# abeytheo/gan-inpainting

Measured on AMD Instinct MI355X. Metric: training images/sec at 256x256 bs=32/GPU, higher is better.
Workload: dtype f16; 1 GPU; wgan_rmse 256x256 bs=32/GPU (BASELINE.json configs[3]): U-Net G (41.8M) + PatchGAN critic, RMSprop 5e-5, clip 0.01, RMSE recon, G update every 5th batch, random-init weights; global_batch=32, parallelism=dp1, compute=fp16 MFMA, fp32 accumulate, fp32 master weights

## Files before the change

### gan-inpainting_amd/backend.py

```python
import ctypes as C
import os
import threading

import torch

_HERE = os.path.dirname(os.path.abspath(__file__))
LIB_PATH = os.environ.get("GI_LIB_PATH") or os.path.join(_HERE, "libganinpaint.so")

GI_F32, GI_F16 = 0, 1
ACT_NONE, ACT_RELU, ACT_LRELU = 0, 1, 2

_vp, _i, _i64, _f, _u64 = C.c_void_p, C.c_int, C.c_int64, C.c_float, C.c_uint64

PROTOTYPES = {
    "gi_last_error": (C.c_char_p, []),
    "gi_version": (_i, []),
    "gi_set_option": (_i, [C.c_char_p, _i]),
    "gi_get_option": (_i, [C.c_char_p, C.POINTER(_i)]),
    "gi_debug_last_kernel": (C.c_char_p, []),
    "gi_debug_fold_count": (_i, []),
    "gi_ctx_create": (_i, [_i, _vp, C.POINTER(_vp)]),
    "gi_ctx_destroy": (_i, [_vp]),
    "gi_ctx_sync": (_i, [_vp]),
    "gi_unet_create": (_i, [_vp, _i, _i, _f, _i, _i, _i, _i, _i, C.POINTER(_vp)]),
    "gi_unet_create_ex": (_i, [_vp, _i, _i, _i, _f, _i, _i, _i, _i, _i, C.POINTER(_vp)]),
    "gi_unet_create_norm": (_i, [_vp, _i, _i, _i, _i, _f, _i, _i, _i, _i, _i, C.POINTER(_vp)]),
    "gi_unet_create_padded": (_i, [_vp, _i, _i, _i, _i, _i, _f, _i, _i, _i, _i, _i, C.POINTER(_vp)]),
    "gi_patchgan_create": (_i, [_vp, _i, _i, _i, _i, _i, _i, C.POINTER(_vp)]),
    "gi_patchgan_create_sn": (_i, [_vp, _i, _i, _i, _i, _i, _i, _i, _i, C.POINTER(_vp)]),
    "gi_net_sn_read": (_i, [_vp, _i, _vp, _vp, _i64]),
    "gi_dcgan_create": (_i, [_vp, _i, _i, _i, _i, _i, C.POINTER(_vp)]),
    "gi_dcgan_debug_forward_convs": (_i, [_vp, _i, _vp, _i]),
    "gi_net_destroy": (_i, [_vp]),
    "gi_net_tensor_count": (_i, [_vp]),
    "gi_net_tensor_desc": (_i, [_vp, _i, C.c_char_p, _i, C.POINTER(_i), C.POINTER(_i64), C.POINTER(_i),
                                C.POINTER(_i64), C.POINTER(_i64)]),
    "gi_net_param_floats": (_i64, [_vp]),
    "gi_net_buffer_floats": (_i64, [_vp]),
    "gi_net_workspace_bytes": (_i64, [_vp]),
    "gi_net_bind": (_i, [_vp, _vp, _vp, _vp, _vp, _i64]),
    "gi_net_sync_weights": (_i, [_vp]),
    "gi_net_set_train": (_i, [_vp, _i]),
    "gi_net_set_inference": (_i, [_vp, _i]),
    "gi_net_set_loss_scale": (_i, [_vp, _f]),
    "gi_net_set_bn_groups": (_i, [_vp, _i]),
    "gi_net_set_dropout_seed": (_i, [_vp, _u64]),
    "gi_net_get_dropout_state": (_i, [_vp, C.POINTER(_u64), C.POINTER(_u64)]),
    "gi_net_set_dropout_state": (_i, [_vp, _u64, _u64]),
    "gi_net_dropout_mask": (_i, [_vp, _i, _i, _vp, _i64]),
    "gi_net_saved_activation": (_i, [_vp, _i, _i, _i, _vp, _i64]),
    "gi_net_debug_nonzero_tickets": (_i, [_vp, _vp]),
    "gi_net_set_dropout_mask": (_i, [_vp, _i, _i, _vp]),
    "gi_net_forward": (_i, [_vp, _i, _vp, _vp, _i]),
    "gi_net_backward": (_i, [_vp, _i, _vp, _vp, _i]),
    "gi_net_backward_phase": (_i, [_vp, _i, _vp, _vp, _i, _i]),
    "gi_net_phase_split": (_i64, [_vp]),
    "gi_net_phase_split2": (_i64, [_vp]),
    "gi_comm_unique_id": (_i, [C.c_char_p]),
    "gi_comm_create": (_i, [C.c_char_p, _i, _i, _i, C.POINTER(_vp)]),
    "gi_comm_destroy": (_i, [_vp]),
    "gi_allreduce_sum_f32": (_i, [_vp, _vp, _i64, _vp]),
    "gi_net_allreduce_grads_async": (_i, [_vp, _vp, _i64, _i64, _vp]),
    "gi_allreduce_wait": (_i, [_vp, _vp, _vp]),
    "gi_patchgan_gradient_penalty": (_i, [_vp, _vp, _i, _f, _vp]),
    "gi_patchgan_gp_saved_activation": (_i, [_vp, _i, _vp, _i64]),
    "gi_interpolate": (_i, [_vp, _vp, _vp, _vp, _i, _i64, _vp]),
    "gi_mask_apply": (_i, [_vp, _vp, _vp, _vp, _vp, _i64, _i]),
    "gi_mask_composite": (_i, [_vp, _vp, _vp, _vp, _vp, _i64]),
    "gi_mul": (_i, [_vp, _vp, _vp, _vp, _i64]),
    "gi_add": (_i, [_vp, _vp, _vp, _vp, _i64, _f]),
    "gi_loss_l1": (_i, [_vp, _vp, _vp, _i64, _vp, _vp, _f, _vp]),
    "gi_loss_rmse": (_i, [_vp, _vp, _vp, _i64, _f, _vp, _vp, _f, _vp]),
    "gi_loss_mse": (_i, [_vp, _vp, _vp, _i64, _vp, _vp, _f, _vp]),
    "gi_loss_local": (_i, [_vp, _vp, _vp, _vp, _i64, _i, _vp, _vp, _f, _vp]),
    "gi_loss_adv": (_i, [_vp, _vp, _i, _i, _f, _vp, _vp, _f]),
    "gi_loss_adv_pair": (_i, [_vp, _vp, _i, _i, _f, _f, _vp, _vp, _vp, _f, _f]),
    "gi_adam_step": (_i, [_vp, _vp, _vp, _vp, _vp, _i64, _f, _f, _f, _f, _i, _f]),
    "gi_rmsprop_step": (_i, [_vp, _vp, _vp, _vp, _i64, _f, _f, _f, _f, _f]),
    "gi_clamp": (_i, [_vp, _vp, _i64, _f, _f]),
    "gi_grad_absmean": (_i, [_vp, _vp, _vp, _vp, _i, _vp]),
    "gi_ssim_scratch_floats": (_i64, [_i, _i, _i, _i, _i]),
    "gi_ssim": (_i, [_vp, _vp, _vp, _i, _i, _i, _i, _i, _vp, _vp, _vp, _vp]),
    "gi_eval_recon_scratch_floats": (_i64, [_i64]),
    "gi_eval_recon": (_i, [_vp, _vp, _vp, _vp, _i64, _f, _vp, _vp, _vp, _vp]),
    "gi_seg_metrics": (_i, [_vp, _vp, _vp, _i, _i, _i64, _vp, _i, _vp, _vp, _vp]),
    "gi_loss_tv": (_i, [_vp, _vp, _i, _i, _i, _f, _vp, _vp, _f, _vp]),
    "gi_loss_cross_entropy": (_i, [_vp, _vp, _vp, _i, _i, _i64, _vp, _i, _vp, _vp, _f, _vp]),
    "gi_vgg19_create": (_i, [_vp, _i, _i, _i, _vp]),
    "gi_vgg19_destroy": (None, [_vp]),
    "gi_vgg19_param_floats": (_i64, [_vp]),
    "gi_vgg19_workspace_bytes": (_i64, [_vp]),
    "gi_vgg19_num_tensors": (_i, [_vp]),
    "gi_vgg19_tensor_desc": (_i, [_vp, _i, _vp, _i, _vp, _vp]),
    "gi_vgg19_bind": (_i, [_vp, _vp, _vp, _i64]),
    "gi_vgg19_sync_weights": (_i, [_vp]),
    "gi_vgg19_perceptual_style": (_i, [_vp, _vp, _vp, _i, _f, _f, _vp, _vp]),
    "gi_vgg19_features": (_i, [_vp, _vp, _i, _i, _vp]),
    "gi_vgg19_grad_workspace_bytes": (_i64, [_vp]),
    "gi_vgg19_bind_grad": (_i, [_vp, _vp, _i64]),
    "gi_vgg19_perceptual_style_grad": (_i, [_vp, _vp, _vp, _i, _f, _f, _vp, _vp, _vp, _f]),
    "gi_vgg19_grad_layer": (_i, [_vp, _i, _vp]),
    "gi_inception_create": (_i, [_vp, _i, _i, _vp]),
    "gi_inception_destroy": (None, [_vp]),
# ... 206 lines not shown
```

### gan-inpainting_amd/csrc/api.hip

```cpp
#include <string.h>

#include <stdlib.h>

#include "common.h"
#include "stat_acc.h"
#include "igemm_plan.h"

static thread_local char g_err[1024] = "";

void gi_set_error(const char* fmt, ...) {
  va_list ap;
  va_start(ap, fmt);
  vsnprintf(g_err, sizeof(g_err), fmt, ap);
  va_end(ap);
}

namespace {
struct OptDesc { const char* name; int dflt; int value; int state; };
inline int opt_load(const int& v) { return __atomic_load_n(&v, __ATOMIC_RELAXED); }
inline void opt_store(int& v, int x) { __atomic_store_n(&v, x, __ATOMIC_RELAXED); }
OptDesc g_opts[GI_OPT_COUNT] = {
  {"GI_IGEMM5", 7, 0, 0}, {"GI_IGEMM6", 1, 0, 0}, {"GI_IGEMM7", 1, 0, 0}, {"GI_IGEMM_FIXUP", 1, 0, 0}, {"GI_IGEMM_VARIANT", 3, 0, 0},
  {"GI_BN_ACC", 1, 0, 0}, {"GI_FUSE_HEAD", 1, 0, 0}, {"GI_HEAD_FAST", 1, 0, 0}, {"GI_BN_BWD_FUSE", 1, 0, 0}, {"GI_BN_BWD_SMALL", 512, 0, 0},
  {"GI_WGRAD2", 1, 0, 0}, {"GI_WGRAD3", 1, 0, 0}, {"GI_IGEMM8", 1, 0, 0}, {"GI_BN_FOLD", 0, 0, 0}, {"GI_C1_FUSED", 1, 0, 0},
  {"GI_WGRAD_STREAM", 1, 0, 0}, {"GI_MASK_BITS", 1, 0, 0}, {"GI_C1W_FUSE", 1, 0, 0}, {"GI_IGEMM7_WAVES", 8, 0, 0},
};
thread_local const char* g_last_kernel = "";
int g_fold_count = 0;
}
void gi_note_fold() { __atomic_fetch_add(&g_fold_count, 1, __ATOMIC_RELAXED); }

int gi_opt(int id) {
  OptDesc& o = g_opts[id];
  if (opt_load(o.state) == 0) {
    const char* e = getenv(o.name);
    opt_store(o.value, e ? atoi(e) : o.dflt);
    __atomic_store_n(&o.state, 1, __ATOMIC_RELEASE);
  }
  return opt_load(o.value);
}
void gi_note_kernel(const char* name) { g_last_kernel = name; }

extern "C" {

int gi_set_option(const char* name, int value) {
  GI_REQUIRE(name, "set_option: null name");
  for (int i = 0; i < GI_OPT_COUNT; ++i)
    if (strcmp(name, g_opts[i].name) == 0) {
      if (value < 0) opt_store(g_opts[i].state, 0);
      else { opt_store(g_opts[i].value, value); __atomic_store_n(&g_opts[i].state, 2, __ATOMIC_RELEASE); }
      return GI_OK;
    }
  gi_set_error("set_option: unknown option '%s'", name);
  return GI_ERR_INVALID;
}
int gi_get_option(const char* name, int* value) {
  GI_REQUIRE(name && value, "get_option: null argument");
  for (int i = 0; i < GI_OPT_COUNT; ++i)
    if (strcmp(name, g_opts[i].name) == 0) { *value = gi_opt(i); return GI_OK; }
  gi_set_error("get_option: unknown option '%s'", name);
  return GI_ERR_INVALID;
}
const char* gi_debug_last_kernel(void) { return g_last_kernel; }
int gi_debug_fold_count(void) { return __atomic_load_n(&g_fold_count, __ATOMIC_RELAXED); }

const char* gi_last_error(void) { return g_err; }
int gi_version(void) { return 100; }

int gi_ctx_create(int device_id, void* hip_stream, gi_ctx** out) {
  GI_REQUIRE(out != nullptr, "ctx_create: out is null");
  int count = 0;
  GI_HIP(hipGetDeviceCount(&count));
  GI_REQUIRE(device_id >= 0 && device_id < count, "ctx_create: device %d not present (%d visible)", device_id, count);
  GI_HIP(hipSetDevice(device_id));
  hipDeviceProp_t prop;
  GI_HIP(hipGetDeviceProperties(&prop, device_id));
  if (strncmp(prop.gcnArchName, "gfx950", 6) != 0) {
    gi_set_error("ctx_create: device %d is %s; this library is built for gfx950 only", device_id, prop.gcnArchName);
    return GI_ERR_UNSUPPORTED;
  }
  gi_ctx* c = new gi_ctx();
  c->device = device_id;
  c->stream = (hipStream_t)hip_stream;
  *out = c;
  return GI_OK;
}
int gi_ctx_destroy(gi_ctx* ctx) {
  if (ctx && ctx->tickets) (void)hipFree(ctx->tickets);
  if (ctx && ctx->absmean_partials) (void)hipFree(ctx->absmean_partials);
  if (ctx && ctx->diffaug_partials) (void)hipFree(ctx->diffaug_partials);
  delete ctx;
  return GI_OK;
}
int gi_ctx_sync(gi_ctx* ctx) {
  GI_REQUIRE(ctx, "ctx_sync: null");
  GI_HIP(hipStreamSynchronize(ctx->stream));
  return GI_OK;
}

static unsigned* ctx_tickets(gi_ctx* ctx) {
  if (!ctx->tickets) {
    if (hipMalloc((void**)&ctx->tickets, GI_IGEMM_TICKETS * 4) != hipSuccess) { ctx->tickets = nullptr; return nullptr; }
    if (hipMemset(ctx->tickets, 0, GI_IGEMM_TICKETS * 4) != hipSuccess) { (void)hipFree(ctx->tickets); ctx->tickets = nullptr; }
  }
  return ctx->tickets;
}

int gi_conv_s2_forward(gi_ctx* ctx, int dtype, const void* in, const void* w_packed, void* out, int n, int H, int W, int cb, int ldin,
                       int ca, int ldout, int relu_in, int act_out, float* ws, int64_t ws_bytes) {
  GI_REQUIRE(ctx && in && w_packed && out, "conv_s2_forward: null pointer");
  GI_REQUIRE(H % 2 == 0 && W % 2 == 0, "conv_s2_forward: H=%d W=%d must be even", H, W);
  IgemmArgs a;
  memset(&a, 0, sizeof(a));
  a.in = in; a.w = w_packed; a.out = out; a.ws = ws; a.ws_bytes = ws_bytes;
  a.tickets = ws ? ctx_tickets(ctx) : nullptr;
  a.n = n; a.Hs = H / 2; a.Ws = W / 2;
  a.cin = cb; a.ldin = ldin; a.cout = ca; a.ldout = ldout;
  a.relu_in = relu_in; a.act_out = act_out;
  return op_igemm(ctx->stream, dtype, 0, a);
}

int gi_convT_s2_forward(gi_ctx* ctx, int dtype, const void* in, const void* w_phase, void* out, int n, int H, int W, int ca, int ldin,
                        int cb, int ldout, int relu_in, int act_out, float* ws, int64_t ws_bytes) {
  GI_REQUIRE(ctx && in && w_phase && out, "convT_s2_forward: null pointer");
  IgemmArgs a;
  memset(&a, 0, sizeof(a));
  a.in = in; a.w = w_phase; a.out = out; a.ws = ws; a.ws_bytes = ws_bytes;
  a.tickets = ws ? ctx_tickets(ctx) : nullptr;
  a.n = n; a.Hs = H; a.Ws = W;
  a.cin = ca; a.ldin = ldin; a.cout = cb; a.ldout = ldout;
  a.relu_in = relu_in; a.act_out = act_out;
  return op_igemm(ctx->stream, dtype, 1, a);
}

static int apply_ex(IgemmArgs& a, const gi_igemm_ex* ex) {
  if (!ex) return GI_OK;
  GI_REQUIRE(ex->relu_cend >= 0 && ex->relu_cend % 64 == 0 && ex->relu_cend <= a.cin, "igemm_ex: relu_cend=%d must be a multiple of 64 within the %d input channels",
             ex->relu_cend, a.cin);
  a.relu_cend = ex->relu_cend;
  a.mask = ex->mask; a.ldmask = ex->ldmask; a.mask_slope = ex->mask_slope;
  a.add = ex->add; a.ldadd = ex->ldadd;
  a.mask_bits = ex->mask ? ex->mask_bits : nullptr;
  a.stat_acc = ex->stat_acc; a.stat_reps = ex->stat_reps; a.stat_pg = ex->stat_pg;
  a.partials = ex->partials;
  a.bwd_x = ex->bwd_x; a.bwd_ldx = ex->bwd_ldx; a.bwd_scale = ex->bwd_scale; a.bwd_shift = ex->bwd_shift; a.bwd_mean = ex->bwd_mean;
  a.bwd_inv = ex->bwd_inv; a.bwd_stride = ex->bwd_stride; a.bwd_slope = ex->bwd_slope; a.bwd_acc = ex->bwd_acc; a.bwd_reps = ex->bwd_reps;
  a.bwd_pg = ex->bwd_pg;
// ... 420 lines not shown
```

### gan-inpainting_amd/csrc/common.h

```cpp
#pragma once
#include <hip/hip_runtime.h>
#include <stdint.h>
#include <stdio.h>
#include <stdarg.h>
#include <mutex>
#include <type_traits>

#include "../../include/ganinpaint.h"

typedef _Float16 half_t;
typedef _Float16 h8_t __attribute__((ext_vector_type(8)));
typedef _Float16 h4_t __attribute__((ext_vector_type(4)));
typedef _Float16 h2_t __attribute__((ext_vector_type(2)));
typedef __fp16 fp16x4_t __attribute__((__vector_size__(4 * sizeof(__fp16))));
typedef float f4_t __attribute__((ext_vector_type(4)));
typedef unsigned int u4_t __attribute__((ext_vector_type(4)));
typedef float f16_t __attribute__((ext_vector_type(16)));

void gi_set_error(const char* fmt, ...);

enum gi_opt_id {
  GI_OPT_IGEMM5 = 0, GI_OPT_IGEMM6, GI_OPT_IGEMM7, GI_OPT_IGEMM_FIXUP, GI_OPT_IGEMM_VARIANT, GI_OPT_BN_ACC, GI_OPT_FUSE_HEAD,
  GI_OPT_HEAD_FAST, GI_OPT_BN_BWD_FUSE, GI_OPT_BN_BWD_SMALL, GI_OPT_WGRAD2, GI_OPT_WGRAD3, GI_OPT_IGEMM8, GI_OPT_BN_FOLD, GI_OPT_C1_FUSED, GI_OPT_WGRAD_STREAM, GI_OPT_MASK_BITS, GI_OPT_C1W_FUSE, GI_OPT_IGEMM7_WAVES, GI_OPT_COUNT
};
int gi_opt(int id);
void gi_note_kernel(const char* name);
void gi_note_fold();
#ifdef GI_ABLATION
#include <stdlib.h>
static inline int gi_tune(const char* env, int dflt) { const char* e = getenv(env); return e ? atoi(e) : dflt; }
#else
#define gi_tune(env, dflt) (dflt)
#endif

template <int N, typename F>
__host__ __device__ __forceinline__ void static_for(F&& f) {
  if constexpr (N > 0) {
    static_for<N - 1>(f);
    f(std::integral_constant<int, N - 1>{});
  }
}

template <int ACT>
__device__ __forceinline__ float gi_act_c(float v) {
  if constexpr (ACT == GI_ACT_RELU) return v > 0.f ? v : 0.f;
  else if constexpr (ACT == GI_ACT_LRELU) return v > 0.f ? v : 0.2f * v;
  else return v;
}
template <typename F>
__device__ __forceinline__ void gi_with_act(int act, F&& f) {
  if (act == GI_ACT_NONE) f(std::integral_constant<int, GI_ACT_NONE>{});
  else if (act == GI_ACT_RELU) f(std::integral_constant<int, GI_ACT_RELU>{});
  else f(std::integral_constant<int, GI_ACT_LRELU>{});
}
template <typename F>
__device__ __forceinline__ void gi_with_bool(bool b, F&& f) {
  if (b) f(std::true_type{});
  else f(std::false_type{});
}
template <int CTRL>
__device__ __forceinline__ float gi_dpp(float v) {
  return __builtin_bit_cast(float, __builtin_amdgcn_update_dpp(0, __builtin_bit_cast(int, v), CTRL, 0xF, 0xF, true));
}
__device__ __forceinline__ float gi_row16_sum(float v) {
  v += gi_dpp<0xB1>(v);
  v += gi_dpp<0x4E>(v);
  v += gi_dpp<0x141>(v);
  v += gi_dpp<0x140>(v);
  return v;
}

__device__ __forceinline__ f4_t gi_ordered_sum_f4(const f4_t* part, int64_t stride, int k0, int k1, f4_t s) {
  int k = k0;
  for (; k + 8 <= k1; k += 8) {
    f4_t v[8];
#pragma unroll
    for (int j = 0; j < 8; ++j) v[j] = part[(int64_t)(k + j) * stride];
#pragma unroll
    for (int j = 0; j < 8; ++j) s += v[j];
  }
  if (k + 4 <= k1) {
    f4_t v[4];
#pragma unroll
    for (int j = 0; j < 4; ++j) v[j] = part[(int64_t)(k + j) * stride];
#pragma unroll
    for (int j = 0; j < 4; ++j) s += v[j];
    k += 4;
  }
  if (k + 2 <= k1) {
    const f4_t v0 = part[(int64_t)k * stride], v1 = part[(int64_t)(k + 1) * stride];
    s += v0;
    s += v1;
    k += 2;
  }
  if (k < k1) s += part[(int64_t)k * stride];
  return s;
}

struct GiDevOnce {
  unsigned long long mask = 0;
  std::mutex mu;
  bool first() {
    int d = 0;
    (void)hipGetDevice(&d);
    const unsigned long long b = 1ull << (d & 63);
    const unsigned long long old = __atomic_fetch_or(&mask, b, __ATOMIC_RELAXED);
    return (old & b) == 0;
  }
  template <typename F>
  hipError_t once(F&& f) {
// ... 291 lines not shown
```

### gan-inpainting_amd/csrc/elementwise.hip

```cpp
#include <stdlib.h>
#include <string.h>

#include "common.h"
#include "stat_acc.h"
#include "bn_acc.h"

namespace {

constexpr int kMaxBlocks = 2048;

template <typename T, int EPC>
__device__ __forceinline__ void load_vec(const char* base, int64_t elem_off, float (&v)[EPC]) {
  if constexpr (std::is_same<T, half_t>::value) {
    const h8_t h = *(const h8_t*)(base + elem_off * 2);
#pragma unroll
    for (int e = 0; e < EPC; ++e) v[e] = (float)h[e];
  } else {
    const f4_t f = *(const f4_t*)(base + elem_off * 4);
#pragma unroll
    for (int e = 0; e < EPC; ++e) v[e] = f[e];
  }
}
template <int EPC>
__device__ __forceinline__ void load_f32(const float* src, float (&v)[EPC]) {
// ... 1372 lines not shown
#define GI_BN_APPLY(T, G) hipLaunchKernelGGL((bn_apply_kernel<T, G, false>), dim3(grid), dim3(256), 0, st, (const char*)x, (char*)y, pixels, c, ldy, coffy, scale, shift, act, (uint8_t*)drop_mask, drop_scale, pg, gstride, fa, (uint64_t)0, (uint32_t)0, (const u4_t*)nullptr, (u4_t*)nullptr, (int64_t)0)
  if (dtype == GI_F16) { if (g2) GI_BN_APPLY(half_t, true); else GI_BN_APPLY(half_t, false); }
  else { if (g2) GI_BN_APPLY(float, true); else GI_BN_APPLY(float, false); }
#undef GI_BN_APPLY
  GI_LAUNCH_CHECK();
  return GI_OK;
}

static void fill_acc_params(BnAccP& fa, const BnAccArgs& b) { gi_fill_acc_params(fa, b); }

int op_bn_finalize_acc(hipStream_t st, int c, const BnAccArgs& b) {
  GI_REQUIRE(b.groups == 1 || b.groups == 2, "bn_finalize_acc: groups=%d", b.groups);
  BnAccP fa;
  fill_acc_params(fa, b);
  hipLaunchKernelGGL(bn_finalize_acc_kernel, dim3((c + 255) / 256), dim3(256), 0, st, fa, c);
  GI_LAUNCH_CHECK();
  return GI_OK;
}

int op_bn_apply_acc(hipStream_t st, int dtype, const void* x, void* y, int64_t pixels, int c, int ldy, int coffy, int act,
                    uint8_t* drop_mask, float drop_scale, uint64_t drop_seed, float drop_p, const BnAccArgs& b,
                    const void* side_src, void* side_dst, int64_t side_bytes) {
  GI_REQUIRE(side_bytes % 16 == 0 && (side_bytes == 0 || (side_src && side_dst)), "bn_apply_acc: side copy of %lld bytes", (long long)side_bytes);
  const int epc = dtype == GI_F16 ? 8 : 4;
  GI_REQUIRE(c % epc == 0 && gi_is_pow2(c / epc) && c / epc <= 256, "bn_apply_acc: c=%d", c);
  GI_REQUIRE(b.groups == 1 || b.groups == 2, "bn_apply_acc: groups=%d", b.groups);
  GI_REQUIRE(pixels % b.groups == 0 && b.count == pixels / b.groups, "bn_apply_acc: %lld pixels, %d populations of %lld", (long long)pixels,
             b.groups, (long long)b.count);
  int grid = nblocks(pixels * (c / epc), 8);
  if (grid > 1024) grid = 1024;
  const bool g2 = b.groups == 2;
  BnAccP fa;
  fill_acc_params(fa, b);
  const size_t lds = (size_t)b.groups * 2 * c * sizeof(float);
  const uint32_t thresh = drop_p > 0.f ? dropout_thresh(drop_p) : 0u;
#define GI_BN_APPLY(T, G) hipLaunchKernelGGL((bn_apply_kernel<T, G, true>), dim3(grid), dim3(256), lds, st, (const char*)x, (char*)y, pixels, c, ldy, coffy, (const float*)nullptr, (const float*)nullptr, act, drop_mask, drop_scale, (int64_t)b.count, 0, fa, drop_seed, thresh, (const u4_t*)side_src, (u4_t*)side_dst, side_bytes / 16)
  if (dtype == GI_F16) { if (g2) GI_BN_APPLY(half_t, true); else GI_BN_APPLY(half_t, false); }
  else { if (g2) GI_BN_APPLY(float, true); else GI_BN_APPLY(float, false); }
#undef GI_BN_APPLY
  GI_LAUNCH_CHECK();
  return GI_OK;
}

static int rows_per_block_for(int64_t pixels, int* blocks_out) {
  int64_t rpb = (pixels + 1023) / 1024;
  if (rpb < 32) rpb = 32;
  *blocks_out = (int)((pixels + rpb - 1) / rpb);
  return (int)rpb;
}

int op_col_stats(hipStream_t st, int dtype, const void* x, int64_t pixels, int c, float* partials, int* rows_out) {
  const int epc = dtype == GI_F16 ? 8 : 4;
  const int Q = c / epc;
  GI_REQUIRE(c % epc == 0 && gi_is_pow2(Q) && Q <= 256, "col_stats: c=%d unsupported", c);
  int blocks;
  const int rpb = rows_per_block_for(pixels, &blocks);
  if (dtype == GI_F16)
    hipLaunchKernelGGL(col_stats_kernel<half_t>, dim3(blocks), dim3(256), 0, st, (const char*)x, pixels, c, partials, rpb);
  else
    hipLaunchKernelGGL(col_stats_kernel<float>, dim3(blocks), dim3(256), 0, st, (const char*)x, pixels, c, partials, rpb);
  GI_LAUNCH_CHECK();
  *rows_out = blocks;
  return GI_OK;
}

int op_bwd_rows_per_block(int64_t pixels) {
  int blocks;
  return rows_per_block_for(pixels, &blocks);
}

static int launch_bwd_reduce(hipStream_t st, int dtype, const BwdP& p, int blocks) {
  const bool need_y = p.g2 != nullptr || p.act != GI_ACT_NONE;
  const bool load_y = need_y && !p.scale;
  const int in = (p.g1 ? 1 : 0) | (p.g2 ? 2 : 0);
  GI_REQUIRE(in != 0, "act_bn_bwd: no upstream gradient");
#define GI_RED(T, IN_, LY_) hipLaunchKernelGGL((act_bn_bwd_reduce_kernel<T, IN_, LY_>), dim3(blocks), dim3(256), 0, st, p)
#define GI_RED_T(IN_, LY_) do { if (dtype == GI_F16) GI_RED(half_t, IN_, LY_); else GI_RED(float, IN_, LY_); } while (0)
  if (in == 1) { if (load_y) GI_RED_T(1, true); else GI_RED_T(1, false); }
  else if (in == 2) { if (load_y) GI_RED_T(2, true); else GI_RED_T(2, false); }
  else { if (load_y) GI_RED_T(3, true); else GI_RED_T(3, false); }
#undef GI_RED_T
#undef GI_RED
  GI_LAUNCH_CHECK();
  return GI_OK;
}

int op_act_bn_bwd(hipStream_t st, int dtype, const ActBnBwdArgs& a) {
  const int epc = dtype == GI_F16 ? 8 : 4;
  const int Q = a.c / epc;
  GI_REQUIRE(a.c % epc == 0 && gi_is_pow2(Q) && Q <= 256, "act_bn_bwd: c=%d unsupported", a.c);
  BwdP p;
  p.g1 = (const char*)a.g1; p.ldg1 = a.ldg1; p.coffg1 = a.coffg1;
  p.g2 = (const char*)a.g2; p.ldg2 = a.ldg2; p.coffg2 = a.coffg2;
  p.y = (const char*)a.y; p.ldy = a.ldy; p.coffy = a.coffy;
  p.x = (const char*)a.x; p.dx = (char*)a.dx;
  p.pixels = a.pixels; p.c = a.c; p.act = a.act; p.drop_scale = a.drop_scale;
  p.gamma = a.gamma; p.mean = a.save_mean; p.inv = a.save_invstd;
  p.partials = a.partials; p.sums = a.sums;
  p.scale = a.has_bn ? a.fwd_scale : nullptr; p.shift = a.has_bn ? a.fwd_shift : nullptr;
  const int groups = (a.groups == 2 && a.has_bn && !a.eval_bn) ? 2 : 1;
  GI_REQUIRE(a.groups <= 1 || groups == 2, "act_bn_bwd: groups=%d needs a train-mode BatchNorm", a.groups);
  GI_REQUIRE(a.pixels % groups == 0, "act_bn_bwd: %lld pixels in %d groups", (long long)a.pixels, groups);
  p.pg = a.pixels / groups; p.stat_stride = a.stat_stride;
  int blocks = 0;
  p.rows_per_block = rows_per_block_for(p.pg, &blocks);
  const int grid2 = nblocks(a.pixels * Q, 4);
  p.acc = nullptr; p.acc_reps = a.acc_reps > 0 ? a.acc_reps : 1; p.dgamma = a.dgamma; p.dbeta = a.dbeta; p.inv_loss_scale = a.inv_loss_scale; p.invM = 1.f / (float)p.pg;
  p.zero_next = nullptr; p.zero_words = 0;
  int small_max = gi_opt(GI_OPT_BN_BWD_SMALL);
  if (small_max > 2048) small_max = 2048;
  if (a.has_bn && !a.eval_bn && groups == 1 && a.pixels <= small_max && !a.reduce_done) {
    p.zero_next = a.acc ? a.zero_next : nullptr; p.zero_words = a.acc ? a.zero_words : 0;
    const int nit = (int)((a.pixels + 255) / 256);
#define GI_SMALL(T) do { if (nit <= 1) hipLaunchKernelGGL((act_bn_bwd_small_kernel<T, 1>), dim3(Q), dim3(256), 0, st, p); \
      else if (nit <= 2) hipLaunchKernelGGL((act_bn_bwd_small_kernel<T, 2>), dim3(Q), dim3(256), 0, st, p); \
      else if (nit <= 4) hipLaunchKernelGGL((act_bn_bwd_small_kernel<T, 4>), dim3(Q), dim3(256), 0, st, p); \
      else hipLaunchKernelGGL((act_bn_bwd_small_kernel<T, 8>), dim3(Q), dim3(256), 0, st, p); } while (0)
    if (dtype == GI_F16) GI_SMALL(half_t); else GI_SMALL(float);
#undef GI_SMALL
    GI_LAUNCH_CHECK();
    return GI_OK;
  }
  if (a.has_bn && a.acc) {
    int grid3 = nblocks(a.pixels * Q, gi_tune("GI_BWD_APPLY_CPT", 8));
    if (grid3 > 1024) grid3 = 1024;
    const size_t lds = (size_t)groups * 5 * a.c * sizeof(float);
    if (!a.eval_bn) {
      GI_REQUIRE(groups == 1 || p.pg % p.rows_per_block == 0, "act_bn_bwd: %lld pixels per group not a multiple of %d rows",
                 (long long)p.pg, p.rows_per_block);
      p.acc = a.acc;
      if (!a.reduce_done) {
        GI_TRY(launch_bwd_reduce(st, dtype, p, blocks * groups));
      }
      p.zero_next = a.zero_next; p.zero_words = a.zero_words;
    } else {
      p.dgamma = nullptr; p.dbeta = nullptr;
    }
    const bool need_y = a.g2 != nullptr || a.act != GI_ACT_NONE;
    const bool load_y = need_y && !p.scale;
    const int in = (a.g1 ? 1 : 0) | (a.g2 ? 2 : 0);
#define GI_APPLY_ACC(T, IN_, LY_, G2_) hipLaunchKernelGGL((act_bn_bwd_apply_acc_kernel<T, IN_, LY_, G2_>), dim3(grid3), dim3(256), lds, st, p)
#define GI_APPLY_ACC_T(IN_, LY_, G2_) do { if (dtype == GI_F16) GI_APPLY_ACC(half_t, IN_, LY_, G2_); else GI_APPLY_ACC(float, IN_, LY_, G2_); } while (0)
    if (in == 1 && !load_y && groups == 2) GI_APPLY_ACC_T(1, false, true);
    else if (in == 1 && !load_y && groups == 1) GI_APPLY_ACC_T(1, false, false);
    else if (in == 3 && !load_y && groups == 1) GI_APPLY_ACC_T(3, false, false);
    else if (in == 2 && !load_y && groups == 1) GI_APPLY_ACC_T(2, false, false);
    else if (in == 2 && load_y && groups == 1) GI_APPLY_ACC_T(2, true, false);
    else if (groups == 2) {
      if (dtype == GI_F16) hipLaunchKernelGGL((act_bn_bwd_apply_kernel<half_t, 2, true>), dim3(grid3), dim3(256), lds, st, p);
      else hipLaunchKernelGGL((act_bn_bwd_apply_kernel<float, 2, true>), dim3(grid3), dim3(256), lds, st, p);
    } else {
      if (dtype == GI_F16) hipLaunchKernelGGL((act_bn_bwd_apply_kernel<half_t, 2, false>), dim3(grid3), dim3(256), lds, st, p);
      else hipLaunchKernelGGL((act_bn_bwd_apply_kernel<float, 2, false>), dim3(grid3), dim3(256), lds, st, p);
    }
#undef GI_APPLY_ACC_T
#undef GI_APPLY_ACC
  } else if (a.has_bn && a.eval_bn) {
    hipLaunchKernelGGL(bwd_sums_kernel, dim3(a.c), dim3(256), 0, st, a.partials, 0, a.c, a.sums, (float*)nullptr, (float*)nullptr, 0.f, 1,
                       a.gamma, a.save_mean, a.save_invstd, p.scale, p.shift, 0, 0.f);
    GI_LAUNCH_CHECK();
    if (dtype == GI_F16) hipLaunchKernelGGL((act_bn_bwd_apply_kernel<half_t, 1, false>), dim3(grid2), dim3(256), 0, st, p);
    else hipLaunchKernelGGL((act_bn_bwd_apply_kernel<float, 1, false>), dim3(grid2), dim3(256), 0, st, p);
  } else if (a.has_bn) {
    GI_REQUIRE(groups == 1 || p.pg % p.rows_per_block == 0, "act_bn_bwd: %lld pixels per group not a multiple of %d rows",
               (long long)p.pg, p.rows_per_block);
    GI_TRY(launch_bwd_reduce(st, dtype, p, blocks * groups));
// ... 334 lines not shown
```

### gan-inpainting_amd/csrc/halo_args.h

```cpp
#pragma once
#include <stdlib.h>

#include "igemm_plan.h"

struct KP5 {
  const char* in;
  const char* w;
  char* out;
  const char* zero;
  const float* bias;
  float* partials;
  unsigned long long* stat_acc; int stat_pg, stat_reps;
  int Hs, Ws, n;
  int TH, TW;
  int tiles_x, tiles_per_img, mtiles;
  int cin, ldin, coffin;
  int cout, ldout, coffout;
  int nchunk;
  int relu_in, relu_cend, act_out;
  int ntiles;
  const char* mask; int ldmask, coffmask; float mask_slope;
  const char* add; int ldadd, coffadd;
  const unsigned long long* mask_bits;
  const float* c1w_img; float* c1w_part; float c1w_scale; int c1w_skip_out;
  const char* bwd_x; int bwd_ldx;
  const float* bwd_scale; const float* bwd_shift; const float* bwd_mean; const float* bwd_inv; int bwd_stride;
  float bwd_slope;
  int bwd_c0, bwd_c;
  unsigned long long* bwd_acc; int bwd_reps; int bwd_pg_tiles;
  int pool;
  int dbg_epi;
};

static inline int fill_halo_args(KP5& kp, const IgemmPlan& p, const IgemmArgs& a) {
  kp = KP5{};
  kp.in = (const char*)a.in; kp.w = (const char*)a.w; kp.out = (char*)a.out; kp.zero = gi_igemm_zero_page();
  if (!kp.zero) { gi_set_error("igemm5: no zero page"); return GI_ERR_HIP; }
  kp.bias = a.bias; kp.partials = a.stat_acc ? nullptr : a.partials;
  kp.stat_acc = a.stat_acc; kp.stat_pg = a.stat_pg; kp.stat_reps = a.stat_reps > 0 ? a.stat_reps : 1;
  kp.Hs = a.Hs; kp.Ws = a.Ws; kp.n = a.n; kp.TH = p.TH; kp.TW = p.TW;
  kp.tiles_x = a.Ws / p.TW; kp.tiles_per_img = kp.tiles_x * (a.Hs / p.TH); kp.mtiles = p.mtiles;
  kp.cin = a.cin; kp.ldin = a.ldin; kp.coffin = a.coffin;
  kp.cout = a.cout; kp.ldout = a.ldout; kp.coffout = a.coffout;
  kp.nchunk = a.cin / 64;
  kp.relu_in = a.relu_in; kp.act_out = a.act_out;
  kp.relu_cend = a.relu_cend > 0 ? a.relu_cend : a.cin;
  kp.ntiles = p.ntiles;
  kp.mask = (const char*)a.mask; kp.ldmask = a.ldmask; kp.coffmask = a.coffmask; kp.mask_slope = a.mask_slope;
  kp.add = a.mask ? (const char*)a.add : nullptr; kp.ldadd = a.ldadd; kp.coffadd = a.coffadd;
  if (p.take_mask_bits) kp.mask_bits = a.mask_bits;
  if (p.take_c1w) { kp.c1w_img = a.c1w_img; kp.c1w_part = a.c1w_part; kp.c1w_scale = a.c1w_scale; kp.c1w_skip_out = a.c1w_skip_out; }
  kp.bwd_c = a.cout;
  if (p.take_bwd) {
    const int64_t px_per_tile = 256 * (p.mode == 0 ? 1 : 4);
    kp.bwd_x = (const char*)a.bwd_x; kp.bwd_ldx = a.bwd_ldx;
    kp.bwd_scale = a.bwd_scale; kp.bwd_shift = a.bwd_shift; kp.bwd_mean = a.bwd_mean; kp.bwd_inv = a.bwd_inv; kp.bwd_stride = a.bwd_stride;
    kp.bwd_slope = a.bwd_slope; kp.bwd_acc = a.bwd_acc; kp.bwd_reps = a.bwd_reps > 0 ? a.bwd_reps : 1;
    kp.bwd_pg_tiles = a.bwd_pg > 0 ? (int)(a.bwd_pg / px_per_tile) : 0;
    if (p.bwd_range) { kp.bwd_c0 = a.bwd_c0; kp.bwd_c = a.bwd_c; }
  }
  kp.pool = p.take_pool ? 1 : 0;
#ifdef GI_ABLATION
  { const char* e = getenv("GI_EPI_DBG"); if (e) kp.dbg_epi = atoi(e); }
#endif
  return GI_OK;
}
```

### gan-inpainting_amd/csrc/igemm3.hip

```cpp
#include <stdlib.h>

#include "common.h"
#include "stat_acc.h"
#include "igemm_plan.h"

namespace {

struct KP3 {
  const char* in;
  const char* w;
  char* out;
  const char* zero;
  const float* bias;
  float* partials;
  unsigned long long* stat_acc; int stat_pg, stat_reps;
  int M, Hs, Ws;
  int cin, ldin, coffin;
  int cout, ldout, coffout;
  int Ktot, nk;
  int relu_in, act_out;
  int relu_cend;
  int Hin, Win, Hout, Wout;
  int mtiles, ntiles;
  int dbg;
};


__device__ __forceinline__ h8_t relu_h8(h8_t v) {
  typedef short s8_t __attribute__((ext_vector_type(8)));
  s8_t h = __builtin_bit_cast(s8_t, v);
  const s8_t z = {0, 0, 0, 0, 0, 0, 0, 0};
  h = __builtin_elementwise_max(h, z);
  return __builtin_bit_cast(h8_t, h);
}

__device__ __forceinline__ void glds16(const char* src, char* lds_wave_base) {
  __builtin_amdgcn_global_load_lds((const __attribute__((address_space(1))) void*)src,
                                   (__attribute__((address_space(3))) void*)lds_wave_base, 16, 0, 0);
}

template <int PHASE, int BN, int NW, int DBG = 0>
__global__ void __launch_bounds__(NW * 64, NW / 4) igemm3_kernel(KP3 p) {
  constexpr int BM = 256, BK = 64;
  constexpr int A_BYTES = BM * 128, B_BYTES = BN * 128, STAGE = A_BYTES + B_BYTES;
  constexpr int NSTG = BN == 256 ? 2 : 3;
  constexpr int AJ = 32 / NW, BJ = (BN / 8) / NW;
  constexpr int WNW = NW / 4;
  constexpr int WN = BN / WNW;
  constexpr int MT = 4, NT = WN / 16;
  constexpr int NTHREADS = NW * 64;
  extern __shared__ __attribute__((aligned(16))) char smem[];

  const int tid = threadIdx.x, lane = tid & 63;
  const int wave = __builtin_amdgcn_readfirstlane(tid >> 6);
  const int wm = wave / WNW, wn = wave % WNW;

  const int nyz = p.ntiles * (PHASE == 1 ? 4 : 1);
  const int bid = blockIdx.x;
  const int xcd = bid & 7, local = bid >> 3;
  const int mt_idx = (local / nyz) * 8 + xcd;
  if (mt_idx >= p.mtiles) return;
  const int yz = local % nyz;
  const int nt_idx = yz % p.ntiles;
  const int ph = yz / p.ntiles;
  const int py = ph >> 1, px = ph & 1;
  const int m0 = mt_idx * BM, n0 = nt_idx * BN;
  const char* wptr = p.w + (PHASE == 1 ? (int64_t)ph * p.cout * p.Ktot * 2 : 0);

  const int lrow = lane >> 3;
  const int lchunk = (lane & 7) ^ (lrow & 7);
  int abase[AJ];
  unsigned amask[AJ];
#pragma unroll
  for (int j = 0; j < AJ; ++j) {
    const int m = m0 + (wave * AJ + j) * 8 + lrow;
    abase[j] = 0;
    amask[j] = 0;
    if (m < p.M) {
      const int x = m % p.Ws;
      const int t = m / p.Ws;
      const int y = t % p.Hs;
      const int n = t / p.Hs;
      if (PHASE == 2) {
        const int y0 = y - 1, x0 = x - 1;
        abase[j] = ((n * p.Hin + y0) * p.Win + x0) * p.ldin + p.coffin;
#pragma unroll
        for (int tt = 0; tt < 9; ++tt) {
          const int iy = y0 + tt / 3, ix = x0 + tt % 3;
          if (iy >= 0 && iy < p.Hin && ix >= 0 && ix < p.Win) amask[j] |= 1u << tt;
        }
      } else if (PHASE) {
        const int y0 = y + py, x0 = x + px;
        abase[j] = ((n * p.Hs + y0) * p.Ws + x0) * p.ldin + p.coffin;
#pragma unroll
        for (int tt = 0; tt < 4; ++tt) {
          const int iy = y0 - (tt >> 1), ix = x0 - (tt & 1);
          if (iy >= 0 && iy < p.Hs && ix >= 0 && ix < p.Ws) amask[j] |= 1u << tt;
        }
      } else {
        const int y0 = 2 * y - 1, x0 = 2 * x - 1;
        abase[j] = ((n * p.Hin + y0) * p.Win + x0) * p.ldin + p.coffin;
#pragma unroll
        for (int tt = 0; tt < 16; ++tt) {
          const int iy = y0 + (tt >> 2), ix = x0 + (tt & 3);
          if (iy >= 0 && iy < p.Hin && ix >= 0 && ix < p.Win) amask[j] |= 1u << tt;
        }
      }
// ... 133 lines not shown
        case 1: if (is) compute(S1{}, S0{}, T1{}); else compute(S1{}, S0{}, T0{}); break;
        default: if (is) compute(S2{}, S1{}, T1{}); else compute(S2{}, S1{}, T0{}); break;
      }
    }
  } else {
    issue(S0{});
    for (int t = 0; t < nk; ++t) {
      asm volatile("s_waitcnt vmcnt(0)" ::: "memory");
      __builtin_amdgcn_s_barrier();
      asm volatile("" ::: "memory");
      const bool is = t + 1 < nk;
      if (t & 1) { if (is) compute(S1{}, S0{}, T1{}); else compute(S1{}, S0{}, T0{}); }
      else { if (is) compute(S0{}, S1{}, T1{}); else compute(S0{}, S1{}, T0{}); }
    }
  }
  asm volatile("s_waitcnt vmcnt(0)" ::: "memory");
  __syncthreads();

  auto out_pixel = [&](int m) -> int {
    if (PHASE != 1) return m;
    const int x = m % p.Ws;
    const int t = m / p.Ws;
    const int y = t % p.Hs;
    const int n = t / p.Hs;
    return (n * p.Hout + 2 * y + py) * p.Wout + 2 * x + px;
  };
  constexpr int SLD = BN + 8;
  half_t* stg = (half_t*)smem;
  float* red = (float*)(smem + (int64_t)BM * SLD * 2);
  const bool stats = p.partials || p.stat_acc;
  gi_with_act(p.act_out, [&](auto ACTc) {
  gi_with_bool(stats, [&](auto STc) {
  gi_with_bool(p.bias != nullptr, [&](auto BIc) {
    constexpr int ACT = decltype(ACTc)::value;
    constexpr bool ST = decltype(STc)::value, BI = decltype(BIc)::value;
#pragma unroll
    for (int nt = 0; nt < NT; ++nt) {
      const int ch = wn * WN + nt * 16 + 4 * lq;
      float bs[4] = {0.f, 0.f, 0.f, 0.f};
      if constexpr (BI) {
#pragma unroll
        for (int r = 0; r < 4; ++r) bs[r] = p.bias[n0 + ch + r];
      }
      float s[4] = {0.f, 0.f, 0.f, 0.f}, q[4] = {0.f, 0.f, 0.f, 0.f};
#pragma unroll
      for (int mt = 0; mt < MT; ++mt) {
        h4_t o;
#pragma unroll
        for (int r = 0; r < 4; ++r) {
          float v = acc[mt][nt][r];
          if constexpr (BI) v += bs[r];
          if constexpr (ST) { s[r] += v; q[r] += v * v; }
          o[r] = (half_t)gi_act_c<ACT>(v);
        }
        *(h4_t*)(stg + (wm * 64 + mt * 16 + lr) * SLD + ch) = o;
      }
      if constexpr (ST) {
#pragma unroll
        for (int r = 0; r < 4; ++r) { s[r] = gi_row16_sum(s[r]); q[r] = gi_row16_sum(q[r]); }
        if (lr == 0) {
#pragma unroll
          for (int r = 0; r < 4; ++r) { red[(wm * BN + ch + r) * 2] = s[r]; red[(wm * BN + ch + r) * 2 + 1] = q[r]; }
        }
      }
    }
  }); }); });
  __syncthreads();
  if ((p.partials || p.stat_acc) && tid < BN) {
    float s = 0.f, q = 0.f;
#pragma unroll
    for (int i = 0; i < 4; ++i) { s += red[(i * BN + tid) * 2]; q += red[(i * BN + tid) * 2 + 1]; }
    if (p.stat_acc) {
      const int grp = (p.stat_pg > 0 && m0 >= p.stat_pg) ? 1 : 0, rep = (mt_idx + ph) & (p.stat_reps - 1);
      gi_stat_add(p.stat_acc, p.cout, rep, grp, 0, n0 + tid, s);
      gi_stat_add(p.stat_acc, p.cout, rep, grp, 1, n0 + tid, q);
    } else {
      const int64_t trow = (int64_t)mt_idx + (int64_t)p.mtiles * ph;
      p.partials[(trow * 2 + 0) * p.cout + n0 + tid] = s;
      p.partials[(trow * 2 + 1) * p.cout + n0 + tid] = q;
    }
  }
  constexpr int CPRO = BN / 8;
  const int oc = tid % CPRO;
#pragma unroll 1
  for (int r = tid / CPRO; r < BM; r += NTHREADS / CPRO) {
    const int m = m0 + r;
    if (m < p.M && !(DBG & 8)) {
      const int64_t o = (int64_t)out_pixel(m) * p.ldout + p.coffout + n0 + oc * 8;
      *(u4_t*)(p.out + o * 2) = *(const u4_t*)((const char*)stg + ((int64_t)r * SLD + oc * 8) * 2);
    }
  }
}

char* g_zero_page[16] = {nullptr};

}

const char* gi_igemm3_zero_page(int dev) {
  if (!g_zero_page[dev & 15]) {
    if (hipMalloc((void**)&g_zero_page[dev & 15], 8192) != hipSuccess) return nullptr;
    if (hipMemset(g_zero_page[dev & 15], 0, 8192) != hipSuccess) return nullptr;
  }
  return g_zero_page[dev & 15];
}

int launch_igemm3(hipStream_t st, const IgemmPlan& p, const IgemmArgs& a) {
  const int mode = p.mode;
  KP3 kp;
  kp.in = (const char*)a.in; kp.w = (const char*)a.w; kp.out = (char*)a.out; kp.zero = gi_igemm_zero_page();
  if (!kp.zero) { gi_set_error("igemm3: no zero page"); return GI_ERR_HIP; }
  kp.bias = a.bias; kp.partials = a.stat_acc ? nullptr : a.partials;
  kp.stat_acc = a.stat_acc; kp.stat_pg = a.stat_pg; kp.stat_reps = a.stat_reps > 0 ? a.stat_reps : 1;
  kp.M = a.n * a.Hs * a.Ws; kp.Hs = a.Hs; kp.Ws = a.Ws;
  kp.cin = a.cin; kp.ldin = a.ldin; kp.coffin = a.coffin;
  kp.cout = a.cout; kp.ldout = a.ldout; kp.coffout = a.coffout;
  kp.Ktot = (mode == 1 ? 4 : (mode == 2 ? 9 : 16)) * a.cin;
  kp.nk = kp.Ktot / 64;
  kp.relu_in = a.relu_in; kp.act_out = a.act_out;
  kp.relu_cend = a.relu_cend > 0 ? a.relu_cend : a.cin;
  kp.dbg = 0;
  if (mode == 1) { kp.Hin = a.Hs; kp.Win = a.Ws; kp.Hout = 2 * a.Hs; kp.Wout = 2 * a.Ws; }
  else if (mode == 2) { kp.Hin = a.Hs; kp.Win = a.Ws; kp.Hout = a.Hs; kp.Wout = a.Ws; }
  else { kp.Hin = 2 * a.Hs; kp.Win = 2 * a.Ws; kp.Hout = a.Hs; kp.Wout = a.Ws; }
  kp.mtiles = p.mtiles;
  kp.ntiles = p.ntiles;
#define GI_K3(V, MODE_, BN_, NAME) case V: return gi_launch_lds<igemm3_kernel<MODE_, BN_, 8>>(dim3(p.grid), 512, p.lds_bytes, p.lds_attr_bytes, st, kp);
#ifdef GI_ABLATION
  { const char* e = getenv("GI_IGEMM3_DBG"); kp.dbg = e ? atoi(e) : 0; }
#define GI_K3D(D_) case D_: return gi_launch_lds<igemm3_kernel<1, 128, 8, D_>>(dim3(p.grid), 512, p.lds_bytes, p.lds_attr_bytes, st, kp);
  if (kp.dbg && p.variant == 1) switch (kp.dbg) {
    GI_K3D(1) GI_K3D(2) GI_K3D(4) GI_K3D(7) GI_K3D(8) GI_K3D(15)
    default: return gi_launch_lds<igemm3_kernel<1, 128, 8, 31>>(dim3(p.grid), 512, p.lds_bytes, p.lds_attr_bytes, st, kp);
  }
#undef GI_K3D
#endif
  switch (p.variant) { GI_IGEMM3_KERNELS(GI_K3) }
#undef GI_K3
  return GI_ERR_INVALID;
}
```

### gan-inpainting_amd/csrc/igemm5.hip

```cpp
#include <stdlib.h>

#include "common.h"
#include "stat_acc.h"
#include "halo_args.h"

namespace {

__device__ __forceinline__ h8_t relu5(h8_t v) {
  typedef short s8_t __attribute__((ext_vector_type(8)));
  s8_t h = __builtin_bit_cast(s8_t, v);
  const s8_t z = {0, 0, 0, 0, 0, 0, 0, 0};
  h = __builtin_elementwise_max(h, z);
  return __builtin_bit_cast(h8_t, h);
}
__device__ __forceinline__ void glds16(const char* src, char* lds_wave_base) {
  __builtin_amdgcn_global_load_lds((const __attribute__((address_space(1))) void*)src,
                                   (__attribute__((address_space(3))) void*)lds_wave_base, 16, 0, 0);
}
__device__ __forceinline__ void blds16(__amdgpu_buffer_rsrc_t rs, unsigned voff, int soff, char* lds_wave_base) {
  __builtin_amdgcn_raw_ptr_buffer_load_lds(rs, (__attribute__((address_space(3))) void*)lds_wave_base, 16, voff, soff, 0, 0);
}
__device__ __forceinline__ void wait_vm(int n) {
  switch (n) {
    case 0: asm volatile("s_waitcnt vmcnt(0)" ::: "memory"); break;
    case 1: asm volatile("s_waitcnt vmcnt(1)" ::: "memory"); break;
    case 2: asm volatile("s_waitcnt vmcnt(2)" ::: "memory"); break;
    case 3: asm volatile("s_waitcnt vmcnt(3)" ::: "memory"); break;
    case 4: asm volatile("s_waitcnt vmcnt(4)" ::: "memory"); break;
    default: asm volatile("s_waitcnt vmcnt(5)" ::: "memory"); break;
  }
}

template <int MODE, int BN>
__device__ __forceinline__ void epilogue5(const KP5& p, f4_t (&acc)[4][BN / 32], char* smem, int tid, int lane, int wm, int wn,
                                          int mt_idx, int nt_idx, int ph, int py, int px, int n0, int img, int y0, int x0, int lgTW) {
  constexpr bool DUAL = MODE == 3;
  constexpr bool PH = MODE == 1 || MODE == 3;
  constexpr int BM = 256, WN = BN / 2, MT = 4, NT = WN / 16;
  const int lr = lane & 15, lq = lane >> 4;
  auto out_pixel = [&](int m) -> int {
    const int ty_l = m >> lgTW, tx_l = m & (p.TW - 1);
    if constexpr (PH) return (img * 2 * p.Hs + 2 * (y0 + ty_l) + py) * (2 * p.Ws) + 2 * (x0 + tx_l) + px;
    else return (img * p.Hs + y0 + ty_l) * p.Ws + x0 + tx_l;
  };
  constexpr int SLD = BN + 8;
  half_t* stg = (half_t*)smem;
  float* red = (float*)(smem + (int64_t)BM * SLD * 2);
  const bool stats = p.partials || p.stat_acc;
  gi_with_act(p.act_out, [&](auto ACTc) {
  gi_with_bool(stats, [&](auto STc) {
  gi_with_bool(p.bias != nullptr, [&](auto BIc) {
    constexpr int ACT = decltype(ACTc)::value;
    constexpr bool ST = decltype(STc)::value, BI = decltype(BIc)::value;
#pragma unroll
    for (int nt = 0; nt < NT; ++nt) {
      const int ch = wn * WN + nt * 16 + 4 * lq;
      float bs[4] = {0.f, 0.f, 0.f, 0.f};
      if constexpr (BI) {
#pragma unroll
        for (int r = 0; r < 4; ++r) bs[r] = p.bias[n0 + (DUAL ? (ch & 63) : ch) + r];
      }
      float s[4] = {0.f, 0.f, 0.f, 0.f}, q[4] = {0.f, 0.f, 0.f, 0.f};
#pragma unroll
      for (int mt = 0; mt < MT; ++mt) {
        h4_t o;
#pragma unroll
        for (int r = 0; r < 4; ++r) {
          float v = acc[mt][nt][r];
          if constexpr (BI) v += bs[r];
          if constexpr (ST) { s[r] += v; q[r] += v * v; }
          o[r] = (half_t)gi_act_c<ACT>(v);
        }
        *(h4_t*)(stg + (wm * 64 + mt * 16 + lr) * SLD + ch) = o;
      }
      if constexpr (ST) {
#pragma unroll
        for (int r = 0; r < 4; ++r) { s[r] = gi_row16_sum(s[r]); q[r] = gi_row16_sum(q[r]); }
        if (lr == 0) {
#pragma unroll
          for (int r = 0; r < 4; ++r) { red[(wm * BN + ch + r) * 2] = s[r]; red[(wm * BN + ch + r) * 2 + 1] = q[r]; }
        }
      }
    }
  }); }); });
  __syncthreads();
  if ((p.partials || p.stat_acc) && tid < BN) {
    float s = 0.f, q = 0.f;
#pragma unroll
    for (int i = 0; i < 4; ++i) { s += red[(i * BN + tid) * 2]; q += red[(i * BN + tid) * 2 + 1]; }
    const int phr = MODE == 1 ? ph : (DUAL ? py * 2 + (tid >> 6) : 0);
    const int col = DUAL ? (tid & 63) : tid;
    if (p.stat_acc) {
      const int grp = (p.stat_pg > 0 && mt_idx * BM >= p.stat_pg) ? 1 : 0, rep = (mt_idx + phr) & (p.stat_reps - 1);
      gi_stat_add(p.stat_acc, p.cout, rep, grp, 0, n0 + col, s);
      gi_stat_add(p.stat_acc, p.cout, rep, grp, 1, n0 + col, q);
    } else {
      const int64_t trow = (int64_t)mt_idx + (int64_t)p.mtiles * phr;
      p.partials[(trow * 2 + 0) * p.cout + n0 + col] = s;
      p.partials[(trow * 2 + 1) * p.cout + n0 + col] = q;
    }
  }
  constexpr int CPRO = BN / 8;
  const int oc = tid % CPRO;
  const bool bwd = !DUAL && p.bwd_acc != nullptr;
  float bsc[8], bsh[8], bmu[8], biv[8], bs[8], bsx[8];
  if (bwd) {
    const int go = (p.bwd_pg_tiles > 0 && mt_idx >= p.bwd_pg_tiles) ? p.bwd_stride : 0;
#pragma unroll
    for (int e = 0; e < 8; ++e) {
      const int ch = go + n0 + oc * 8 + e;
      bsc[e] = p.bwd_scale[ch]; bsh[e] = p.bwd_shift[ch]; bmu[e] = p.bwd_mean[ch]; biv[e] = p.bwd_inv[ch];
      bs[e] = bsx[e] = 0.f;
    }
  }
  constexpr int NR = BM / (512 / CPRO);
  int opxs[NR];
  u4_t mk[NR], ad[NR], xs[NR];
  const int och = n0 + (DUAL ? (oc & 7) : oc) * 8;
#pragma unroll
  for (int k = 0; k < NR; ++k) {
    const int r = tid / CPRO + k * (512 / CPRO);
    opxs[k] = out_pixel(r) + (DUAL ? (oc >> 3) : 0);
    const int64_t opx = opxs[k];
    if (p.mask) mk[k] = *(const u4_t*)(p.mask + (opx * p.ldmask + p.coffmask + och) * 2);
    if (p.mask && p.add) ad[k] = *(const u4_t*)(p.add + (opx * p.ldadd + p.coffadd + och) * 2);
    if (bwd) xs[k] = *(const u4_t*)(p.bwd_x + (opx * p.bwd_ldx + och) * 2);
  }
#pragma unroll
  for (int k = 0; k < NR; ++k) {
    const int r = tid / CPRO + k * (512 / CPRO);
    const int64_t opx = opxs[k];
    const int64_t o = opx * p.ldout + p.coffout + och;
    u4_t v = *(const u4_t*)((const char*)stg + ((int64_t)r * SLD + oc * 8) * 2);
    if (bwd) {
      const h8_t xv = __builtin_bit_cast(h8_t, xs[k]);
      const h8_t gv = __builtin_bit_cast(h8_t, v);
#pragma unroll
      for (int e = 0; e < 8; ++e) {
        const float xf = (float)xv[e];
        const float dz = (float)gv[e] * (fmaf(xf, bsc[e], bsh[e]) > 0.f ? 1.f : p.bwd_slope);
        bs[e] += dz;
        bsx[e] = fmaf(dz, (xf - bmu[e]) * biv[e], bsx[e]);
      }
    }
    if (p.mask) {
      const h8_t m = __builtin_bit_cast(h8_t, mk[k]);
      h8_t hv = __builtin_bit_cast(h8_t, v);
      if (p.add) {
        const h8_t a8 = __builtin_bit_cast(h8_t, ad[k]);
#pragma unroll
        for (int e = 0; e < 8; ++e) {
          const bool pos = (float)m[e] > 0.f;
          const float g = (float)hv[e] + (pos ? (float)a8[e] : 0.f);
          hv[e] = (half_t)(pos ? g : g * p.mask_slope);
        }
      } else {
#pragma unroll
        for (int e = 0; e < 8; ++e) hv[e] = (float)m[e] > 0.f ? hv[e] : (half_t)((float)hv[e] * p.mask_slope);
      }
      v = __builtin_bit_cast(u4_t, hv);
    }
#ifdef GI_ABLATION
    if (p.dbg_epi & 1) { *(u4_t*)(p.out + ((o * 2) & 0xFFF0)) = v; continue; }
#endif
    *(u4_t*)(p.out + o * 2) = v;
  }
  if (bwd) {
    static_assert(DUAL || CPRO == 16 || CPRO == 8, "CPRO");
#pragma unroll
    for (int e = 0; e < 8; ++e) {
#pragma unroll
      for (int off = CPRO; off < 64; off <<= 1) { bs[e] += __shfl_xor(bs[e], off); bsx[e] += __shfl_xor(bsx[e], off); }
    }
    __syncthreads();
    float* fold = (float*)smem;
    if (lane < CPRO) {
#pragma unroll
      for (int e = 0; e < 8; ++e) { fold[((tid >> 6) * BN + oc * 8 + e) * 2] = bs[e]; fold[((tid >> 6) * BN + oc * 8 + e) * 2 + 1] = bsx[e]; }
    }
    __syncthreads();
    if (tid < BN) {
      float s = 0.f, q = 0.f;
#pragma unroll
      for (int w = 0; w < 8; ++w) { s += fold[(w * BN + tid) * 2]; q += fold[(w * BN + tid) * 2 + 1]; }
      const int grp = (p.bwd_pg_tiles > 0 && mt_idx >= p.bwd_pg_tiles) ? 1 : 0, rep = (mt_idx + (MODE == 1 ? ph : 0)) & (p.bwd_reps - 1);
      gi_stat_add(p.bwd_acc, p.cout, rep, grp, 0, n0 + tid, s);
      gi_stat_add(p.bwd_acc, p.cout, rep, grp, 1, n0 + tid, q);
    }
  }
}

template <int MODE, int BN>
__global__ void __launch_bounds__(512, 2) igemm5_kernel(KP5 p) {
  constexpr bool DUAL = MODE == 3;
  constexpr bool PH = MODE == 1 || MODE == 3;
  constexpr int NQ = MODE == 0 ? 4 : 1;
  constexpr int NTAP = MODE == 2 ? 9 : 4;
  constexpr int PAD = MODE == 2 ? 2 : 1;
  constexpr int PADX = DUAL ? 2 : PAD;
  static_assert(!DUAL || BN == 128, "dual-px mode: 2 x 64 columns");
  constexpr int BM = 256, BK = 64, NW = 8;
  constexpr int AJ = MODE == 2 ? 6 : 5;
  constexpr int A_ROWS = AJ * 64, A_BYTES = A_ROWS * 128;
  constexpr int B_BYTES = BN * 128;
  constexpr int A_OFF = 0, B_OFF = 2 * A_BYTES;
  constexpr int BJ = (BN / 8) / NW;
  constexpr int WN = BN / 2, MT = 4, NT = WN / 16;
  extern __shared__ __attribute__((aligned(16))) char smem[];

  const int tid = threadIdx.x, lane = tid & 63;
  const int wave = __builtin_amdgcn_readfirstlane(tid >> 6);
  const int wm = wave >> 1, wn = wave & 1;

  const int nyz = p.ntiles * (DUAL ? 2 : (PH ? 4 : 1));
  const int bid = blockIdx.x;
  const int xcd = bid & 7, local = bid >> 3;
  const int mt_idx = (local / nyz) * 8 + xcd;
  if (mt_idx >= p.mtiles) return;
  const int yz = local % nyz;
  const int nt_idx = yz % p.ntiles;
  const int ph = yz / p.ntiles;
  const int py = DUAL ? ph : (ph >> 1), px = DUAL ? 0 : (ph & 1);
  const int n0 = nt_idx * (DUAL ? 64 : BN);
  const int img = mt_idx / p.tiles_per_img, trem = mt_idx % p.tiles_per_img;
  const int y0 = (trem / p.tiles_x) * p.TH, x0 = (trem % p.tiles_x) * p.TW;
  const int HC = p.TW + PADX, HR = p.TH + PAD;
  const int Ktot2 = (PH ? 4 : (MODE == 2 ? 9 : 16)) * p.cin * 2;
  const int64_t phase_bytes = (int64_t)p.cout * Ktot2;
  const char* wptr = p.w + (MODE == 1 ? ph * phase_bytes : (DUAL ? (py * 2) * phase_bytes : 0));
  const int Win = 2 * p.Ws, Hin = 2 * p.Hs;

  const int lrow = lane >> 3;
  const int lchunk = (lane & 7) ^ (lrow & 7);
  const char* pa[AJ];
  unsigned amask[AJ];
#pragma unroll
  for (int j = 0; j < AJ; ++j) {
    const int r = (wave * AJ + j) * 8 + lrow;
    const int hr = r / HC, hc = r - hr * HC;
    amask[j] = 0;
    if constexpr (MODE != 0) {
      const int iy = y0 + (PH ? py : 0) - 1 + hr, ix = x0 + (MODE == 1 ? px : 0) - 1 + hc;
      const bool ok = hr < HR && iy >= 0 && iy < p.Hs && ix >= 0 && ix < p.Ws;
      pa[j] = ok ? p.in + ((int64_t)((img * p.Hs + iy) * p.Ws + ix) * p.ldin + p.coffin) * 2 + lchunk * 16 : p.zero + lchunk * 16;
    } else {
      const int iy0 = 2 * (y0 + hr), ix0 = 2 * (x0 + hc);
      pa[j] = p.in + ((int64_t)((img * Hin + iy0) * Win + ix0) * p.ldin + p.coffin) * 2 + lchunk * 16;
#pragma unroll
// ... 306 lines not shown
#pragma unroll
    for (int j = 0; j < AJ; ++j) va[j] = next_a ? voffA[QN][j] : OOB;
    static_for<NTAP>([&](auto TAPc) {
      constexpr int tap = decltype(TAPc)::value;
      const int s = c * NTAP + tap;
      constexpr int ptap = (tap + 3) & 3;
      constexpr int nwait = BJ + (ptap == 0 ? 3 : (ptap == 1 ? 2 : 0));
      if constexpr (nwait == 1) asm volatile("s_waitcnt vmcnt(1)" ::: "memory");
      else if constexpr (nwait == 2) asm volatile("s_waitcnt vmcnt(2)" ::: "memory");
      else if constexpr (nwait == 3) asm volatile("s_waitcnt vmcnt(3)" ::: "memory");
      else if constexpr (nwait == 4) asm volatile("s_waitcnt vmcnt(4)" ::: "memory");
      else asm volatile("s_waitcnt vmcnt(5)" ::: "memory");
      if constexpr ((DBG & 16) == 0) __builtin_amdgcn_s_barrier();
      asm volatile("" ::: "memory");
      Frag f1;
      unsigned vb[BJ];
#pragma unroll
      for (int j = 0; j < BJ; ++j) vb[j] = s + 3 < nsteps ? voffB[j] : OOB;
      auto issue_piece = [&](auto IDX) {
        constexpr int idx = decltype(IDX)::value;
        constexpr int NM = 2 * MT * NT;
        if constexpr ((DBG & 1) != 0) return;
        if constexpr (tap == 0) {
          if constexpr (idx == NM / 4) blds16(rsA, va[0], chunk_n * (BK * 2), smem + A_OFF + (BUF ^ 1) * A_BYTES + (wave * AJ + 0) * 1024);
          if constexpr (idx == NM / 4 + 2) blds16(rsA, va[1], chunk_n * (BK * 2), smem + A_OFF + (BUF ^ 1) * A_BYTES + (wave * AJ + 1) * 1024);
          if constexpr (idx == NM / 4 + 4) blds16(rsA, va[2], chunk_n * (BK * 2), smem + A_OFF + (BUF ^ 1) * A_BYTES + (wave * AJ + 2) * 1024);
        } else if constexpr (tap == 1) {
          if constexpr (idx == NM / 4) blds16(rsA, va[3], chunk_n * (BK * 2), smem + A_OFF + (BUF ^ 1) * A_BYTES + (wave * AJ + 3) * 1024);
          if constexpr (idx == NM / 4 + 3) blds16(rsA, va[4], chunk_n * (BK * 2), smem + A_OFF + (BUF ^ 1) * A_BYTES + (wave * AJ + 4) * 1024);
        }
        static_for<BJ>([&](auto Jc) {
          constexpr int j = decltype(Jc)::value;
          if constexpr (idx == NM - 2 - (BJ - 1 - j) * 2) {
            if constexpr (tap == 0) issue_b(vb, chunk, QT{}, I3{}, Jc);
            else issue_b(vb, chunk_n, QNT{}, std::integral_constant<int, tap - 1>{}, Jc);
          }
        });
      };
      static_for<MT * NT>([&](auto IDX) {
        constexpr int idx = decltype(IDX)::value, mt = idx / NT, nt = idx % NT;
        if constexpr (nt == 0) relu_a(f0.a[mt], rmin);
        if constexpr ((DBG & 2) != 0) { asm volatile("" :: "v"(f0.a[mt])); asm volatile("" :: "v"(f0.b[nt])); }
        else acc[mt][nt] = __builtin_amdgcn_mfma_f32_16x16x32_f16(f0.b[nt], f0.a[mt], acc[mt][nt], 0, 0, 0);
        if constexpr (RSTEP * (idx / RSTEP) == idx && idx / RSTEP < MT + NT)
          read_one(BUFT{}, TAPc, I1{}, std::integral_constant<int, rorder(idx / RSTEP)>{}, f1);
        issue_piece(IDX);
        __builtin_amdgcn_sched_barrier(0);
      });
      static_for<MT * NT>([&](auto IDX) {
        constexpr int idx = decltype(IDX)::value, mt = idx / NT, nt = idx % NT;
        if constexpr (nt == 0) relu_a(f1.a[mt], rmin);
        if constexpr ((DBG & 2) != 0) { asm volatile("" :: "v"(f1.a[mt])); asm volatile("" :: "v"(f1.b[nt])); }
        else acc[mt][nt] = __builtin_amdgcn_mfma_f32_16x16x32_f16(f1.b[nt], f1.a[mt], acc[mt][nt], 0, 0, 0);
        if constexpr (RSTEP * (idx / RSTEP) == idx && idx / RSTEP < MT + NT) {
          using RI = std::integral_constant<int, rorder(idx / RSTEP)>;
          if constexpr (tap < 3) read_one(BUFT{}, std::integral_constant<int, tap + 1>{}, I0{}, RI{}, f0);
          else read_one(BUFN{}, I0{}, I0{}, RI{}, f0);
        }
        issue_piece(std::integral_constant<int, idx + MT * NT>{});
        __builtin_amdgcn_sched_barrier(0);
      });
    });
  };

  if constexpr (MODE == 0) {
    for (int c = 0; c < ngroups; c += 4) { group(c, I0{}); group(c + 1, I1{}); group(c + 2, I2{}); group(c + 3, I3{}); }
  } else {
    int c = 0;
    for (; c + 1 < ngroups; c += 2) { group(c, I0{}); group(c + 1, I1{}); }
    if (c < ngroups) group(c, I0{});
  }
  asm volatile("s_waitcnt vmcnt(0)" ::: "memory");
  __syncthreads();
  asm volatile("" ::: "memory");
  if constexpr ((DBG & 64) != 0) {
    float t = 0.f;
#pragma unroll
    for (int i = 0; i < MT; ++i)
#pragma unroll
      for (int j = 0; j < NT; ++j) t += acc[i][j][0] + acc[i][j][1] + acc[i][j][2] + acc[i][j][3];
    if (t == 12345.678f) p.out[0] = 1;
    return;
  }
  epilogue5<MODE, BN>(p, acc, smem, tid, lane, wm, wn, mt_idx, nt_idx, ph, py, px, n0, img, y0, x0, lgTW);
}

}

int launch_igemm5(hipStream_t st, const IgemmPlan& p, const IgemmArgs& a) {
  KP5 kp;
  GI_TRY(fill_halo_args(kp, p, a));
  const dim3 grid(p.grid);
#define GI_K5(V, MODE_, BN_, NAME) case V: return gi_launch_lds<igemm5_kernel<MODE_, BN_>>(grid, 512, p.lds_bytes, p.lds_attr_bytes, st, kp);
#define GI_K6(V, MODE_, BN_, RELU_, NAME) case V: return gi_launch_lds<igemm6_kernel<MODE_, BN_, RELU_>>(grid, 512, p.lds_bytes, p.lds_attr_bytes, st, kp);
  if (p.family == GI_FAM_IGEMM5 && p.variant < 6) switch (p.variant) { GI_IGEMM5_KERNELS(GI_K5) }
  if (p.family == GI_FAM_IGEMM6) {
#ifdef GI_ABLATION
    const char* e = getenv("GI_IGEMM6_DBG"); const int dbg = e ? atoi(e) : 0;
#define GI_K6D(D_) case D_: return gi_launch_lds<igemm6_kernel<1, 128, true, D_>>(grid, 512, p.lds_bytes, p.lds_attr_bytes, st, kp);
    if (dbg && p.variant == 3) switch (dbg) {
      GI_K6D(1) GI_K6D(2) GI_K6D(4) GI_K6D(8) GI_K6D(16) GI_K6D(3) GI_K6D(5) GI_K6D(6) GI_K6D(7) GI_K6D(23) GI_K6D(32) GI_K6D(39)
      GI_K6D(64) GI_K6D(96) GI_K6D(225) GI_K6D(231)
      default: return gi_launch_lds<igemm6_kernel<1, 128, true, 9>>(grid, 512, p.lds_bytes, p.lds_attr_bytes, st, kp);
    }
#undef GI_K6D
#endif
    switch (p.variant) { GI_IGEMM6_KERNELS(GI_K6) }
  }
  switch (p.variant) { GI_IGEMM5_DUAL_KERNEL(GI_K5) }
#undef GI_K5
#undef GI_K6
  return GI_ERR_INVALID;
}
```

### gan-inpainting_amd/csrc/igemm8.hip

```cpp
#include <stdlib.h>

#include "common.h"
#include "stat_acc.h"
#include "halo_args.h"

namespace {

__device__ __forceinline__ void blds16(__amdgpu_buffer_rsrc_t rs, unsigned voff, int soff, char* lds_wave_base) {
  __builtin_amdgcn_raw_ptr_buffer_load_lds(rs, (__attribute__((address_space(3))) void*)lds_wave_base, 16, voff, soff, 0, 0);
}

template <int MODE, int BN, bool BITS>
__device__ __forceinline__ void epilogue8(const KP5& p, f4_t (&acc)[4][BN / 16], char* smem, int tid, int lane, int wave, int mt_idx,
                                          int ph, int py, int px, int n0, int img, int y0, int x0, int lgTW) {
  constexpr bool DUAL = MODE == 3;
  constexpr bool PH = MODE == 1 || MODE == 3;
  constexpr int BM = 256, MT = 4, NT = BN / 16;
  const int lr = lane & 15, lq = lane >> 4;
  auto out_pixel = [&](int m) -> int {
    const int ty_l = m >> lgTW, tx_l = m & (p.TW - 1);
    if constexpr (PH) return (img * 2 * p.Hs + 2 * (y0 + ty_l) + py) * (2 * p.Ws) + 2 * (x0 + tx_l) + px;
    else return (img * p.Hs + y0 + ty_l) * p.Ws + x0 + tx_l;
  };
  constexpr int SLD = BN + 8;
  half_t* stg = (half_t*)smem;
  float* red = (float*)(smem + (int64_t)BM * SLD * 2);
  const bool stats = p.partials || p.stat_acc;
  float c1w_x[BITS ? 4 : 1][8];
  if constexpr (BITS) {
    if (p.c1w_part) {
      const int Himg = 4 * p.Hs, Wimg = 4 * p.Ws;
      const int tap = lane & 15, kq = lane >> 4, ky = tap >> 2, kx = tap & 3;
      const float* ximg = p.c1w_img + (int64_t)img * Himg * Wimg;
#pragma unroll
      for (int bi = 0; bi < 4; ++bi) {
        const int b = wave + 4 * bi;
        const int P = b & 1, mrow = (b >> 1) * 32 + 8 * kq;
        const int iy = 4 * (y0 + (mrow >> lgTW)) + 2 * py - 1 + ky;
        const bool yok = iy >= 0 && iy < Himg;
        const float* rowp = ximg + (int64_t)(yok ? iy : 0) * Wimg;
        const int ix0 = 4 * (x0 + (mrow & (p.TW - 1))) + 2 * P - 1 + kx;
#pragma unroll
        for (int j = 0; j < 8; ++j) {
          const int ix = ix0 + 4 * j;
          const bool ok = yok && ix >= 0 && ix < Wimg;
          const float a = rowp[ok ? ix : 0];
          c1w_x[bi][j] = ok ? a : 0.f;
        }
      }
    }
  }
  if constexpr (BITS) {
    if (p.mask_bits) {
      u4_t mb[MT];
#pragma unroll
      for (int mt = 0; mt < MT; ++mt) mb[mt] = *(const u4_t*)(p.mask_bits + out_pixel(wave * 64 + mt * 16 + lr));
#pragma unroll
      for (int nt = 0; nt < NT; ++nt) {
        const int ch = nt * 16 + 4 * lq;
#pragma unroll
        for (int mt = 0; mt < MT; ++mt) {
          const int t = (int)(mb[mt][nt >> 1] >> ((nt & 1) * 16 + 4 * lq));
          h4_t o;
#pragma unroll
          for (int r = 0; r < 4; ++r) {
            const float v = acc[mt][nt][r];
            const int pos = (t << (31 - r)) >> 31;
            o[r] = (half_t)__builtin_bit_cast(float, (__builtin_bit_cast(int, v) & pos) | (__builtin_bit_cast(int, v * p.mask_slope) & ~pos));
          }
          *(h4_t*)(stg + (wave * 64 + mt * 16 + lr) * SLD + ch) = o;
        }
      }
    }
  }
  auto acc_loop = [&](auto ACTc, auto st, auto bi) {
    constexpr int ACT = decltype(ACTc)::value;
    constexpr bool CT = !std::is_same<decltype(st), bool>::value;
#pragma unroll
    for (int nt = 0; nt < NT; ++nt) {
      const int ch = nt * 16 + 4 * lq;
      float bs[4] = {0.f, 0.f, 0.f, 0.f};
      if (bi) {
#pragma unroll
        for (int r = 0; r < 4; ++r) bs[r] = p.bias[n0 + (DUAL ? (ch & 63) : ch) + r];
      }
      float s[4] = {0.f, 0.f, 0.f, 0.f}, q[4] = {0.f, 0.f, 0.f, 0.f};
#pragma unroll
      for (int mt = 0; mt < MT; ++mt) {
        h4_t o;
#pragma unroll
        for (int r = 0; r < 4; ++r) {
          float v = acc[mt][nt][r];
          if constexpr (CT) {
            if (bi) v += bs[r];
            if (st) { s[r] += v; q[r] += v * v; }
// ... 28 lines not shown
  if ((p.partials || p.stat_acc) && tid < BN) {
    float s = 0.f, q = 0.f;
#pragma unroll
    for (int i = 0; i < 4; ++i) { s += red[(i * BN + tid) * 2]; q += red[(i * BN + tid) * 2 + 1]; }
    const int phr = MODE == 1 ? ph : (DUAL ? py * 2 + (tid >> 6) : 0);
    const int col = DUAL ? (tid & 63) : tid;
    if (p.stat_acc) {
      const int grp = (p.stat_pg > 0 && mt_idx * BM >= p.stat_pg) ? 1 : 0, rep = (mt_idx + phr) & (p.stat_reps - 1);
      gi_stat_add(p.stat_acc, p.cout, rep, grp, 0, n0 + col, s);
      gi_stat_add(p.stat_acc, p.cout, rep, grp, 1, n0 + col, q);
    } else {
      const int64_t trow = (int64_t)mt_idx + (int64_t)p.mtiles * phr;
      p.partials[(trow * 2 + 0) * p.cout + n0 + col] = s;
      p.partials[(trow * 2 + 1) * p.cout + n0 + col] = q;
    }
  }
  constexpr int CPRO = BN / 8;
  const int oc = tid % CPRO;
  const bool bwd = !DUAL && p.bwd_acc != nullptr && n0 >= p.bwd_c0 && n0 < p.bwd_c0 + p.bwd_c;
  const int bn0 = n0 - p.bwd_c0;
  float bsc[8], bsh[8], bmu[8], biv[8], bs[8], bsx[8];
  if (bwd) {
    const int go = (p.bwd_pg_tiles > 0 && mt_idx >= p.bwd_pg_tiles) ? p.bwd_stride : 0;
#pragma unroll
    for (int e = 0; e < 8; ++e) {
      const int ch = go + bn0 + oc * 8 + e;
      bsc[e] = p.bwd_scale[ch]; bsh[e] = p.bwd_shift[ch]; bmu[e] = p.bwd_mean[ch]; biv[e] = p.bwd_inv[ch];
      bs[e] = bsx[e] = 0.f;
    }
  }
  if constexpr (MODE == 2) {
    if (p.pool) {
      constexpr int RPQ = 256 / CPRO;
#pragma unroll
      for (int k = 0; k < 64 / RPQ; ++k) {
        const int r = tid / CPRO + k * RPQ;
        const int m = (2 * (r >> 4)) * 32 + 2 * (r & 15);
        const char* sp = (const char*)stg + ((int64_t)m * SLD + oc * 8) * 2;
        const h8_t a = *(const h8_t*)sp, b = *(const h8_t*)(sp + SLD * 2), c = *(const h8_t*)(sp + 32 * SLD * 2), d = *(const h8_t*)(sp + 33 * SLD * 2);
        const h8_t v = __builtin_elementwise_max(__builtin_elementwise_max(a, b), __builtin_elementwise_max(c, d));
        const int64_t opx = ((int64_t)img * (p.Hs >> 1) + (y0 >> 1) + (r >> 4)) * (p.Ws >> 1) + (x0 >> 1) + (r & 15);
        *(h8_t*)(p.out + (opx * p.ldout + n0 + oc * 8) * 2) = v;
      }
      return;
    }
  }
  constexpr int RP = 256 / CPRO;
  const int och = n0 + (DUAL ? (oc & 7) : oc) * 8;
  bool copied = false;
  if constexpr (BITS) {
    if (p.c1w_part && p.c1w_skip_out && !p.add) copied = true;
    if (p.mask_bits && p.add) {
      constexpr int NB = 4;
#pragma unroll 1
      for (int h = 0; h < BM / (RP * NB); ++h) {
        int opxs[NB], mbyte[NB];
        u4_t ad[NB];
#pragma unroll
        for (int k = 0; k < NB; ++k) {
          const int r = tid / CPRO + (h * NB + k) * RP;
          opxs[k] = out_pixel(r) + (oc >> 3);
          mbyte[k] = ((const unsigned char*)p.mask_bits)[(int64_t)opxs[k] * 8 + (oc & 7)];
          ad[k] = *(const u4_t*)(p.add + ((int64_t)opxs[k] * p.ldadd + p.coffadd + och) * 2);
        }
#pragma unroll
        for (int k = 0; k < NB; ++k) {
          const int r = tid / CPRO + (h * NB + k) * RP;
          u4_t v = *(const u4_t*)((const char*)stg + ((int64_t)r * SLD + oc * 8) * 2);
          const int b = mbyte[k];
          u4_t a8 = ad[k];
#pragma unroll
          for (int i = 0; i < 4; ++i) {
            const unsigned lo = (unsigned)((b << (31 - 2 * i)) >> 31) & 0xFFFFu, hi = (unsigned)((b << (30 - 2 * i)) >> 31) & 0xFFFF0000u;
            a8[i] &= lo | hi;
          }
          v = __builtin_bit_cast(u4_t, __builtin_bit_cast(h8_t, v) + __builtin_bit_cast(h8_t, a8));
          if (p.c1w_part) *(u4_t*)((char*)stg + ((int64_t)r * SLD + oc * 8) * 2) = v;
          if (!p.c1w_skip_out) *(u4_t*)(p.out + ((int64_t)opxs[k] * p.ldout + p.coffout + och) * 2) = v;
        }
      }
      copied = true;
    }
  }
  if constexpr (!DUAL && MODE != 2) {
    if (bwd && !p.mask) {
      constexpr int NB = 4;
#pragma unroll 1
      for (int h = 0; h < BM / (RP * NB); ++h) {
        int opxs[NB];
        u4_t xs[NB];
#pragma unroll
        for (int k = 0; k < NB; ++k) {
          opxs[k] = out_pixel(tid / CPRO + (h * NB + k) * RP);
          xs[k] = *(const u4_t*)(p.bwd_x + ((int64_t)opxs[k] * p.bwd_ldx + och - p.bwd_c0) * 2);
        }
#pragma unroll
        for (int k = 0; k < NB; ++k) {
          const int r = tid / CPRO + (h * NB + k) * RP;
          const u4_t v = *(const u4_t*)((const char*)stg + ((int64_t)r * SLD + oc * 8) * 2);
          const h8_t xv = __builtin_bit_cast(h8_t, xs[k]);
          const h8_t gv = __builtin_bit_cast(h8_t, v);
#pragma unroll
          for (int e = 0; e < 8; ++e) {
            const float xf = (float)xv[e];
            const float dz = (float)gv[e] * (fmaf(xf, bsc[e], bsh[e]) > 0.f ? 1.f : p.bwd_slope);
            bs[e] += dz;
            bsx[e] = fmaf(dz, (xf - bmu[e]) * biv[e], bsx[e]);
          }
          *(u4_t*)(p.out + ((int64_t)opxs[k] * p.ldout + p.coffout + och) * 2) = v;
        }
      }
      copied = true;
    }
  }
  constexpr int NR = 8;
#pragma unroll 1
  for (int h = 0; h < (copied ? 0 : BM / (RP * NR)); ++h) {
    int opxs[NR];
    u4_t mk[NR], ad[NR], xs[NR];
#pragma unroll
    for (int k = 0; k < NR; ++k) {
      const int r = tid / CPRO + (h * NR + k) * RP;
      opxs[k] = out_pixel(r) + (DUAL ? (oc >> 3) : 0);
      const int64_t opx = opxs[k];
#ifdef GI_ABLATION
      if (p.mask && (p.dbg_epi & 2)) mk[k] = *(const u4_t*)(p.mask + (((opx * p.ldmask + p.coffmask + och) * 2) & 0xFFF0));
      else
#endif
      if (BITS && p.mask_bits) {}
      else if (p.mask) mk[k] = *(const u4_t*)(p.mask + (opx * p.ldmask + p.coffmask + och) * 2);
      if (!(BITS && p.mask_bits) && p.mask && p.add) ad[k] = *(const u4_t*)(p.add + (opx * p.ldadd + p.coffadd + och) * 2);
      if (bwd) xs[k] = *(const u4_t*)(p.bwd_x + (opx * p.bwd_ldx + och - p.bwd_c0) * 2);
    }
#pragma unroll
    for (int k = 0; k < NR; ++k) {
      const int r = tid / CPRO + (h * NR + k) * RP;
      const int64_t opx = opxs[k];
      const int64_t o = opx * p.ldout + p.coffout + och;
      u4_t v = *(const u4_t*)((const char*)stg + ((int64_t)r * SLD + oc * 8) * 2);
      if (bwd) {
        const h8_t xv = __builtin_bit_cast(h8_t, xs[k]);
        const h8_t gv = __builtin_bit_cast(h8_t, v);
#pragma unroll
        for (int e = 0; e < 8; ++e) {
          const float xf = (float)xv[e];
          const float dz = (float)gv[e] * (fmaf(xf, bsc[e], bsh[e]) > 0.f ? 1.f : p.bwd_slope);
          bs[e] += dz;
          bsx[e] = fmaf(dz, (xf - bmu[e]) * biv[e], bsx[e]);
        }
      }
      if (BITS && p.mask_bits) {
      } else if (p.mask) {
        const h8_t m = __builtin_bit_cast(h8_t, mk[k]);
        h8_t hv = __builtin_bit_cast(h8_t, v);
        if (p.add) {
          const h8_t a8 = __builtin_bit_cast(h8_t, ad[k]);
#pragma unroll
          for (int e = 0; e < 8; ++e) {
            const bool pos = (float)m[e] > 0.f;
            const float g = (float)hv[e] + (pos ? (float)a8[e] : 0.f);
            hv[e] = (half_t)(pos ? g : g * p.mask_slope);
          }
        } else {
#pragma unroll
          for (int e = 0; e < 8; ++e) hv[e] = (float)m[e] > 0.f ? hv[e] : (half_t)((float)hv[e] * p.mask_slope);
        }
        v = __builtin_bit_cast(u4_t, hv);
      }
#ifdef GI_ABLATION
      if (p.dbg_epi & 1) { *(u4_t*)(p.out + ((o * 2) & 0xFFF0)) = v; continue; }
#endif
      *(u4_t*)(p.out + o * 2) = v;
    }
  }
  if constexpr (BITS) {
    if (p.c1w_part) {
      __syncthreads();
      const int tap = lane & 15, kq = lane >> 4;
      const int tq = tap >> 2, tp = tap & 3;
      f4_t wacc[4];
#pragma unroll
      for (int nt = 0; nt < 4; ++nt) wacc[nt] = f4_t{0.f, 0.f, 0.f, 0.f};
#pragma unroll
      for (int bi = 0; bi < 4; ++bi) {
        const int b = wave + 4 * bi;
        const int P = b & 1, m0 = (b >> 1) * 32;
        h8_t af;
#pragma unroll
        for (int j = 0; j < 8; ++j) af[j] = (half_t)c1w_x[bi][j];
#pragma unroll
        for (int nt = 0; nt < 4; ++nt) {
          const char* b_lo = (const char*)stg + ((m0 + 8 * kq + tq) * SLD + P * 64 + nt * 16 + 4 * tp) * 2;
          const char* b_hi = b_lo + 4 * SLD * 2;
          fp16x4_t lo = __builtin_amdgcn_ds_read_tr16_b64_v4f16((__attribute__((address_space(3))) fp16x4_t*)b_lo);
          fp16x4_t hi = __builtin_amdgcn_ds_read_tr16_b64_v4f16((__attribute__((address_space(3))) fp16x4_t*)b_hi);
          const h4_t l4 = __builtin_bit_cast(h4_t, lo), h4 = __builtin_bit_cast(h4_t, hi);
          const h8_t bf = h8_t{l4[0], l4[1], l4[2], l4[3], h4[0], h4[1], h4[2], h4[3]};
          wacc[nt] = __builtin_amdgcn_mfma_f32_16x16x32_f16(af, bf, wacc[nt], 0, 0, 0);
        }
      }
      __syncthreads();
      float* wred = (float*)smem;
#pragma unroll
      for (int nt = 0; nt < 4; ++nt)
#pragma unroll
        for (int r = 0; r < 4; ++r) wred[wave * 1024 + (nt * 16 + (lane & 15)) * 16 + 4 * (lane >> 4) + r] = wacc[nt][r];
      __syncthreads();
      float* part = p.c1w_part + (int64_t)blockIdx.x * 1024;
      for (int i = tid; i < 1024; i += 256) part[i] = ((wred[i] + wred[1024 + i]) + (wred[2048 + i] + wred[3072 + i])) * p.c1w_scale;
    }
  }
  if (bwd) {
#pragma unroll
    for (int e = 0; e < 8; ++e) {
#pragma unroll
      for (int off = CPRO; off < 64; off <<= 1) { bs[e] += __shfl_xor(bs[e], off); bsx[e] += __shfl_xor(bsx[e], off); }
    }
    __syncthreads();
    float* fold = (float*)smem;
    if (lane < CPRO) {
#pragma unroll
      for (int e = 0; e < 8; ++e) { fold[(wave * BN + oc * 8 + e) * 2] = bs[e]; fold[(wave * BN + oc * 8 + e) * 2 + 1] = bsx[e]; }
    }
    __syncthreads();
    if (tid < BN) {
      float s = 0.f, q = 0.f;
#pragma unroll
      for (int w = 0; w < 4; ++w) { s += fold[(w * BN + tid) * 2]; q += fold[(w * BN + tid) * 2 + 1]; }
      const int grp = (p.bwd_pg_tiles > 0 && mt_idx >= p.bwd_pg_tiles) ? 1 : 0, rep = (mt_idx + (MODE == 1 ? ph : 0)) & (p.bwd_reps - 1);
      gi_stat_add(p.bwd_acc, p.bwd_c, rep, grp, 0, bn0 + tid, s);
      gi_stat_add(p.bwd_acc, p.bwd_c, rep, grp, 1, bn0 + tid, q);
    }
  }
}

template <int MODE, bool RELU, int DBG = 0, int BN = 128>
__global__ void __launch_bounds__(256, 2) igemm8_kernel(KP5 p) {
  static_assert(BN == 128 || (BN == 64 && MODE != 3), "64-column tiles: not with both px phases in one tile");
  static_assert(MODE >= 0 && MODE <= 3, "modes 0 (stride-2 gather), 1 (phase), 2 (3x3 / s1), 3 (both px phases)");
  static_assert(!(MODE == 2 && RELU), "the 3x3 mode has no fused input ReLU");
  constexpr bool DUAL = MODE == 3;
  constexpr bool PH = MODE == 1 || MODE == 3;
  constexpr int NQ = MODE == 0 ? 4 : 1;
  constexpr int NTAP = MODE == 2 ? 9 : 4;
  constexpr int PADX = (DUAL || MODE == 2) ? 2 : 1, PADY = MODE == 2 ? 2 : 1;
  constexpr int BK = 32, NW = 4;
  constexpr int AJ = MODE == 2 ? 6 : 5;
  constexpr int APIECES = MODE == 2 ? 22 : AJ * NW;
  constexpr int AHEAD = 3;
  constexpr int A_BYTES = APIECES * 1024;
  constexpr int B_BYTES = BN * 64;
  constexpr int A_OFF = 0, B_OFF = 2 * A_BYTES;
  constexpr int BJ = (BN / 16) / NW;
  constexpr int MT = 4, NT = BN / 16, NH = NT / 2;
  constexpr int SP = NT == 8 ? 2 : 1;
  constexpr unsigned OOB = 0x80000000u;
  extern __shared__ __attribute__((aligned(16))) char smem[];

  const int tid = threadIdx.x, lane = tid & 63;
  const int wave = __builtin_amdgcn_readfirstlane(tid >> 6);

  const int nyz = p.ntiles * (DUAL ? 2 : (PH ? 4 : 1));
  const int bid = blockIdx.x;
  const int xcd = bid & 7, local = bid >> 3;
  const int mt_idx = (local / nyz) * 8 + xcd;
  if (mt_idx >= p.mtiles) return;
  const int yz = local % nyz;
  const int nt_idx = yz % p.ntiles;
  const int ph = yz / p.ntiles;
  const int py = DUAL ? ph : (ph >> 1), px = DUAL ? 0 : (ph & 1);
  const int n0 = nt_idx * (DUAL ? 64 : BN);
  const int img = mt_idx / p.tiles_per_img, trem = mt_idx % p.tiles_per_img;
  const int y0 = (trem / p.tiles_x) * p.TH, x0 = (trem % p.tiles_x) * p.TW;
  const int HC = p.TW + PADX, HR = p.TH + PADY;
  const int Ktot2 = (PH ? 4 : (MODE == 2 ? 9 : 16)) * p.cin * 2;
  const int64_t phase_bytes = (int64_t)p.cout * Ktot2;
  const int Win = 2 * p.Ws, Hin = 2 * p.Hs;

  const int64_t in_bytes = (int64_t)p.n * (MODE == 0 ? 4 : 1) * p.Hs * p.Ws * p.ldin * 2;
  const __amdgpu_buffer_rsrc_t rsA = __builtin_amdgcn_make_buffer_rsrc((void*)p.in, 0, (int)in_bytes, 0x00020000);
  const char* wbase = p.w + (MODE == 1 ? ph * phase_bytes : (DUAL ? (py * 2) * phase_bytes : 0));
  const __amdgpu_buffer_rsrc_t rsB = __builtin_amdgcn_make_buffer_rsrc((void*)wbase, 0, (int)(DUAL ? 2 * phase_bytes : phase_bytes), 0x00020000);

  const int lrow = lane >> 2, lc = lane & 3;
  unsigned voffA[NQ][AJ];
  auto piece_of = [&](int j) -> int {
    if constexpr (MODE == 2) { const int P = j * NW + wave; return P < APIECES ? P : P - NW; }
    else return wave * AJ + j;
  };
#pragma unroll
  for (int j = 0; j < AJ; ++j) {
    const int r = piece_of(j) * 16 + lrow;
    const int hr = r / HC, hc = r - hr * HC;
    const int cb = (lc ^ ((r >> 1) & 3)) * 16;
    if constexpr (MODE != 0) {
      const int iy = y0 + py - 1 + hr, ix = x0 + (MODE == 1 ? px : 0) - 1 + hc;
      const bool ok = hr < HR && iy >= 0 && iy < p.Hs && ix >= 0 && ix < p.Ws;
      voffA[0][j] = ok ? (unsigned)((((img * p.Hs + iy) * p.Ws + ix) * p.ldin + p.coffin) * 2 + cb) : OOB;
    } else {
#pragma unroll
      for (int q = 0; q < 4; ++q) {
        const int iy = 2 * (y0 + hr) - (q >> 1), ix = 2 * (x0 + hc) - (q & 1);
        const bool ok = hr < HR && iy >= 0 && iy < Hin && ix >= 0 && ix < Win;
        voffA[q][j] = ok ? (unsigned)((((img * Hin + iy) * Win + ix) * p.ldin + p.coffin) * 2 + cb) : OOB;
      }
    }
  }
  unsigned voffB[BJ];
#pragma unroll
  for (int j = 0; j < BJ; ++j) {
    const int rb = (wave * BJ + j) * 16 + lrow;
    const int cb = (lc ^ ((rb >> 1) & 3)) * 16;
    if constexpr (DUAL) voffB[j] = (unsigned)((rb >> 6) * phase_bytes + (int64_t)(n0 + (rb & 63)) * Ktot2 + cb);
    else voffB[j] = (unsigned)((int64_t)(n0 + rb) * Ktot2 + cb);
  }

  const int lr = lane & 15, lq = lane >> 4;
  const int lgTW = 31 - __builtin_clz(p.TW);
  int rdA[MT][MODE == 2 ? 1 : NTAP];
  int rdA2[DUAL ? MT : 1][2];
// ... 127 lines not shown
          if constexpr (idx == NM / 4 + 3) blds16(rsA, va[4], chunk_n * (BK * 2), smem + A_OFF + (BUF ^ 1) * A_BYTES + (wave * AJ + 4) * 1024);
        }
        static_for<BJ>([&](auto Jc) {
          constexpr int j = decltype(Jc)::value;
          if constexpr (idx == NM - 2 - (BJ - 1 - j) * 2) {
            if constexpr (MODE == 2) {
              if constexpr (tap + AHEAD < NTAP) issue_b(vb, chunk, QT{}, std::integral_constant<int, tap + AHEAD>{}, Jc, istg);
              else issue_b(vb, chunk_n, QNT{}, std::integral_constant<int, tap + AHEAD - NTAP>{}, Jc, istg);
            } else {
              if constexpr (tap == 0) issue_b(vb, chunk, QT{}, I3{}, Jc, istg);
              else issue_b(vb, chunk_n, QNT{}, std::integral_constant<int, tap - 1>{}, Jc, istg);
            }
          }
        });
      };
      constexpr int CUR = DUAL ? 0 : ((PAR0 + tap) & 1);
      const int rdBs = rdB + stg * B_BYTES, rdBn = rdB + nstg * B_BYTES;
      constexpr int OTH = DUAL ? 1 : (CUR ^ 1);
      static_for<MT * NH>([&](auto IDX) {
        constexpr int idx = decltype(IDX)::value, mt = idx / NH, nt = idx % NH;
        if constexpr (nt == 0) relu_a(fa[CUR][mt], rmin);
        if constexpr ((DBG & 2) != 0) { asm volatile("" :: "v"(fa[CUR][mt])); asm volatile("" :: "v"(fb[nt])); }
        else acc[mt][nt] = __builtin_amdgcn_mfma_f32_16x16x32_f16(fb[nt], fa[CUR][mt], acc[mt][nt], 0, 0, 0);
        if constexpr (idx % SP == 0) {
          constexpr int k = idx / SP;
          if constexpr (!DUAL) {
            if constexpr (k < NH) fb[NH + k] = ldsr(rdBs + (NH + k) * 1024);
          } else {
            if constexpr (k == 0) fa[1][0] = ldsr(rd_px1(0, TAPc) + BUF * A_BYTES);
            else if constexpr (k <= NH) fb[NH + k - 1] = ldsr(rdBs + (NH + k - 1) * 1024);
            else fa[1][k - NH] = ldsr(rd_px1(k - NH, TAPc) + BUF * A_BYTES);
          }
        }
        issue_piece(IDX);
        __builtin_amdgcn_sched_barrier(0);
      });
      static_for<MT * NH>([&](auto IDX) {
        constexpr int idx = decltype(IDX)::value, mt = idx / NH, nt = NH + idx % NH;
        constexpr int HS = DUAL ? 1 : CUR;
        if constexpr (DUAL && nt == NH) relu_a(fa[1][mt], rmin);
        if constexpr ((DBG & 2) != 0) { asm volatile("" :: "v"(fa[HS][mt])); asm volatile("" :: "v"(fb[nt])); }
        else acc[mt][nt] = __builtin_amdgcn_mfma_f32_16x16x32_f16(fb[nt], fa[HS][mt], acc[mt][nt], 0, 0, 0);
        if constexpr (idx % SP == 0) {
          constexpr int k = idx / SP;
          constexpr int NXT = DUAL ? 0 : OTH;
          constexpr int ntap = (tap + 1) % NTAP;
          constexpr int nbuf = tap < NTAP - 1 ? BUF : (BUF ^ 1);
          using NT_ = std::integral_constant<int, ntap>;
          if constexpr (k == 0) fa[NXT][0] = ldsr(addrA(0, NT_{}) + nbuf * A_BYTES);
          else if constexpr (k <= NH) fb[k - 1] = ldsr(rdBn + (k - 1) * 1024);
          else if constexpr (k < NH + MT) fa[NXT][k - NH] = ldsr(addrA(k - NH, NT_{}) + nbuf * A_BYTES);
        }
        issue_piece(std::integral_constant<int, idx + MT * NH>{});
        __builtin_amdgcn_sched_barrier(0);
      });
    });
  };

  if constexpr (MODE == 0) {
    for (int cp = 0; 2 * cp < nchunk; ++cp) {
      const int c = cp * 8, a = 2 * cp, b = 2 * cp + 1;
      group(c + 0, I0{}, I0{}, I0{}, a, b); group(c + 1, I1{}, I0{}, I1{}, b, a);
      group(c + 2, I0{}, I1{}, I1{}, a, b); group(c + 3, I1{}, I1{}, I2{}, b, a);
      group(c + 4, I0{}, I2{}, I2{}, a, b); group(c + 5, I1{}, I2{}, I3{}, b, a);
      group(c + 6, I0{}, I3{}, I3{}, a, b); group(c + 7, I1{}, I3{}, I0{}, b, a + 2);
    }
  } else {
    int c = 0;
    for (; c + 1 < ngroups; c += 2) { group(c, I0{}, I0{}, I0{}, c, c + 1); group(c + 1, I1{}, I0{}, I0{}, c + 1, c + 2); }
    if (c < ngroups) group(c, I0{}, I0{}, I0{}, c, c + 1);
  }
  asm volatile("s_waitcnt vmcnt(0)" ::: "memory");
  __syncthreads();
  asm volatile("" ::: "memory");
  if constexpr ((DBG & 32) != 0) {
    float t = 0.f;
#pragma unroll
    for (int i = 0; i < MT; ++i)
#pragma unroll
      for (int j = 0; j < NT; ++j) t += acc[i][j][0] + acc[i][j][1] + acc[i][j][2] + acc[i][j][3];
    if (t == 12345.678f) p.out[0] = 1;
    return;
  }
  epilogue8<MODE, BN, (MODE == 3 && !RELU)>(p, acc, smem, tid, lane, wave, mt_idx, ph, py, px, n0, img, y0, x0, lgTW);
}

}

int launch_igemm8(hipStream_t st, const IgemmPlan& p, const IgemmArgs& a) {
  KP5 kp;
  GI_TRY(fill_halo_args(kp, p, a));
  const dim3 grid(p.grid);
#define GI_K8(V, MODE_, RELU_, BN_, NAME) case V: return gi_launch_lds<igemm8_kernel<MODE_, RELU_, 0, BN_>>(grid, 256, p.lds_bytes, p.lds_attr_bytes, st, kp);
#ifdef GI_ABLATION
  const char* e = getenv("GI_IGEMM8_DBG"); const int dbg = e ? atoi(e) : 0;
#define GI_K8D(M_, R_, D_) case D_: return gi_launch_lds<igemm8_kernel<M_, R_, D_>>(grid, 256, p.lds_bytes, p.lds_attr_bytes, st, kp);
  if (dbg && p.variant == 3) switch (dbg) {
    GI_K8D(1, true, 1) GI_K8D(1, true, 2) GI_K8D(1, true, 4) GI_K8D(1, true, 8) GI_K8D(1, true, 16) GI_K8D(1, true, 32) GI_K8D(1, true, 5)
    GI_K8D(1, true, 7) GI_K8D(1, true, 6) GI_K8D(1, true, 3) GI_K8D(1, true, 39) GI_K8D(1, true, 13)
    default: return gi_launch_lds<igemm8_kernel<1, true, 15>>(grid, 256, p.lds_bytes, p.lds_attr_bytes, st, kp);
  }
  const char* e0 = getenv("GI_IGEMM8_DBG0"); const int dbg0 = e0 ? atoi(e0) : 0;
  if (dbg0 && p.variant == 0) switch (dbg0) {
    GI_K8D(0, false, 1) GI_K8D(0, false, 2) GI_K8D(0, false, 4) GI_K8D(0, false, 16) GI_K8D(0, false, 32) GI_K8D(0, false, 5) GI_K8D(0, false, 7)
    default: return gi_launch_lds<igemm8_kernel<0, false, 39>>(grid, 256, p.lds_bytes, p.lds_attr_bytes, st, kp);
  }
#undef GI_K8D
#endif
  switch (p.variant) { GI_IGEMM8_KERNELS(GI_K8) }
#undef GI_K8
  return GI_ERR_INVALID;
}
```

### gan-inpainting_amd/csrc/igemm_plan.h

```cpp
#pragma once
#include "common.h"

enum { GI_FAM_GENERIC = 0, GI_FAM_IGEMM3, GI_FAM_IGEMM5, GI_FAM_IGEMM6, GI_FAM_IGEMM7, GI_FAM_IGEMM8 };

struct IgemmPlan {
  int family;
  int variant;
  int mode, bn;
  bool dual, relu;
  int nw, nstg, pf;
  int BM; bool half_n;
  int splitk, kt_per_split;
  bool fixup, finish_launch, atomics_ws;
  bool fold, take_mask, take_mask_bits, take_c1w, take_bwd, bwd_range, take_pool, stat_to_acc;
  int TH, TW, mtiles, ntiles, grid, lds_bytes, lds_attr_bytes, ntiles_out;
  int finish_rows, finish_blocks;
  const char* name;
};
int gi_igemm_plan(int dtype, int mode, const IgemmArgs& a, IgemmPlan* p);

void gi_igemm_returns(const IgemmPlan& p, IgemmArgs& a);

int launch_igemm(hipStream_t st, int dtype, const IgemmPlan& p, const IgemmArgs& a);
int launch_igemm3(hipStream_t st, const IgemmPlan& p, const IgemmArgs& a);
int launch_igemm5(hipStream_t st, const IgemmPlan& p, const IgemmArgs& a);
int launch_igemm7(hipStream_t st, const IgemmPlan& p, const IgemmArgs& a);
int launch_igemm8(hipStream_t st, const IgemmPlan& p, const IgemmArgs& a);
const char* gi_igemm3_zero_page(int dev);
static inline const char* gi_igemm_zero_page() { int dev = 0; return hipGetDevice(&dev) == hipSuccess ? gi_igemm3_zero_page(dev) : nullptr; }

#define GI_IGEMM3_KERNELS(X)  \
  X(0, 0, 128, "igemm3<0,128>") X(1, 1, 128, "igemm3<1,128>") X(2, 2, 128, "igemm3<2,128>") \
  X(3, 0, 64, "igemm3<0,64>") X(4, 1, 64, "igemm3<1,64>") X(5, 2, 64, "igemm3<2,64>")
#define GI_IGEMM5_KERNELS(X)  \
  X(0, 0, 128, "igemm5<0,128>") X(1, 1, 128, "igemm5<1,128>") X(2, 2, 128, "igemm5<2,128>") \
  X(3, 0, 64, "igemm5<0,64>") X(4, 1, 64, "igemm5<1,64>") X(5, 2, 64, "igemm5<2,64>")
#define GI_IGEMM5_DUAL_KERNEL(X) X(6, 3, 128, "igemm5<3,128>")
#define GI_IGEMM6_KERNELS(X)  \
  X(0, 0, 128, false, "igemm6<0,128>") X(2, 1, 128, false, "igemm6<1,128>") X(3, 1, 128, true, "igemm6<1,128,relu>") \
  X(4, 0, 64, false, "igemm6<0,64>") X(6, 1, 64, false, "igemm6<1,64>") X(7, 1, 64, true, "igemm6<1,64,relu>") \
  X(8, 3, 128, false, "igemm6<3,128>") X(9, 3, 128, true, "igemm6<3,128,relu>")
#define GI_IGEMM7_KERNELS(X)  \
  X(0, 0, 128, "igemm7<0,128>") X(1, 1, 128, "igemm7<1,128>") X(2, 0, 64, "igemm7<0,64>") X(3, 1, 64, "igemm7<1,64>")
#define GI_IGEMM7_FOLD_NAMES(X) X(4, 0, 128, "igemm7<0,128>+bn") X(5, 1, 128, "igemm7<1,128>+bn") X(6, 0, 64, "igemm7<0,64>+bn") X(7, 1, 64, "igemm7<1,64>+bn")
#define GI_IGEMM8_KERNELS(X)  \
  X(7, 2, false, 64, "igemm8<2,64>") X(0, 0, false, 128, "igemm8<0>") X(1, 0, true, 128, "igemm8<0,relu>") X(2, 1, false, 128, "igemm8<1>") \
  X(3, 1, true, 128, "igemm8<1,relu>") X(4, 3, false, 128, "igemm8<3>") X(5, 3, true, 128, "igemm8<3,relu>") X(6, 2, false, 128, "igemm8<2>")
```

### gan-inpainting_amd/csrc/igemm_plan.hip

```cpp
#include "igemm_plan.h"

namespace {

constexpr int NEXT = 1;

#define GI_NAME3(V, A, B, NAME) case V: return NAME;
#define GI_NAME4(V, A, B, C, NAME) case V: return NAME;
#define GI_NAME_FN(FN, ROWS) const char* FN(int variant) { switch (variant) { ROWS } return ""; }
GI_NAME_FN(name3, GI_IGEMM3_KERNELS(GI_NAME3))
GI_NAME_FN(name5, GI_IGEMM5_KERNELS(GI_NAME3) GI_IGEMM5_DUAL_KERNEL(GI_NAME3))
GI_NAME_FN(name6, GI_IGEMM6_KERNELS(GI_NAME4))
GI_NAME_FN(name7, GI_IGEMM7_KERNELS(GI_NAME3) GI_IGEMM7_FOLD_NAMES(GI_NAME3))
GI_NAME_FN(name8, GI_IGEMM8_KERNELS(GI_NAME4))

int plan_halo(int mode, const IgemmArgs& a, IgemmPlan& p) {
  if (!gi_is_pow2(a.Ws) || a.Ws < 8) return NEXT;
  const int TW = a.Ws < 32 ? a.Ws : 32, TH = 256 / TW;
  if (a.Hs % TH != 0) return NEXT;
  if (mode == 2 ? (TH + 2) * (TW + 2) > 384 : (TH + 1) * (TW + ((mode == 1 && a.cout % 128 != 0) ? 2 : 1)) > 320) return NEXT;
  int BN = (a.cout % 128 == 0) ? 128 : 64;
  const int nph = mode == 1 ? 4 : 1;
  const int mtiles = a.n * (a.Ws / TW) * (a.Hs / TH);
  if (mode != 2 && mtiles * (a.cout / BN) * nph < 128) return NEXT;
  if (mode == 0 && BN == 128 && mtiles * (a.cout / BN) < 256) {
    if (gi_tune("GI_IGEMM5_NARROW", 1)) BN = 64;
  }
  const bool dual = mode == 1 && BN == 64;
  const int64_t in_px = (int64_t)a.n * a.Hs * a.Ws * (mode == 0 ? 4 : 1), out_px = (int64_t)a.n * a.Hs * a.Ws * (mode == 1 ? 4 : 1);
  GI_REQUIRE(in_px * a.ldin < (1ll << 31) && out_px * a.ldout < (1ll << 31), "igemm5: tensor too large for 32-bit offsets");
  GI_REQUIRE(!a.stat_acc || a.stat_pg == 0 || a.stat_pg % (a.Hs * a.Ws) == 0, "igemm5: stat_pg=%d must be whole images", a.stat_pg);
  if (a.mask) {
    GI_REQUIRE(a.ldmask % 8 == 0 && a.coffmask % 8 == 0 && out_px * a.ldmask < (1ll << 31), "igemm5: mask layout");
    GI_REQUIRE(!a.add || (a.ldadd % 8 == 0 && a.coffadd % 8 == 0 && out_px * a.ldadd < (1ll << 31)), "igemm5: add layout");
  }
  p.take_mask = a.mask != nullptr;
  p.mode = dual ? 3 : mode; p.bn = BN; p.dual = dual; p.relu = a.relu_in != 0;
  p.TH = TH; p.TW = TW; p.mtiles = mtiles; p.ntiles = a.cout / BN;
  p.grid = ((mtiles + 7) / 8) * 8 * p.ntiles * (dual ? 2 : nph);
  p.ntiles_out = mtiles * nph;
  p.stat_to_acc = a.stat_acc != nullptr;
  const int BNk = dual ? 128 : BN;
  const int epi = 256 * (BNk + 8) * 2 + 4 * BNk * 8;
  const int use6 = gi_opt(GI_OPT_IGEMM6), use8 = use6 ? gi_opt(GI_OPT_IGEMM8) : 0;
  const bool fits31 = in_px * a.ldin * 2 < (1ll << 31) && (int64_t)a.cout * (mode == 1 ? 4 : (mode == 2 ? 9 : 16)) * a.cin * 2 * (dual ? 2 : 1) < (1ll << 31);
  const bool take8 = use8 && (mode != 2 || (TW == 32 && !a.relu_in)) && (dual || BN == 128 || mode == 2) && a.cin % (mode == 0 ? 64 : 32) == 0 && TW >= 16 &&
      fits31 && !(mode == 0 && a.relu_in) && (use8 >= 2 || p.grid >= gi_tune("GI_IGEMM8_MINGRID", 512));
  p.bwd_range = a.bwd_c > 0 && (a.bwd_c0 != 0 || a.bwd_c != a.cout);
  if (a.bwd_acc && !a.mask && mode != 2 && a.cout % 128 == 0 && BN == 128 && (!p.bwd_range || (take8 && a.bwd_c0 % 128 == 0 && a.bwd_c % 128 == 0 && a.bwd_c0 + a.bwd_c <= a.cout))) {
    const int64_t px_per_tile = 256 * (mode == 1 ? 4 : 1);
    GI_REQUIRE(a.bwd_ldx % 8 == 0 && out_px * a.bwd_ldx < (1ll << 31) && (a.bwd_pg == 0 || a.bwd_pg % px_per_tile == 0) && a.coffout == 0,
               "igemm5: fused BatchNorm-backward reduction: layout");
    p.take_bwd = true;
  }
  if (take8) {
    if (mode == 2 && a.pool2 && !a.mask && !a.stat_acc && !a.partials) {
      GI_REQUIRE(a.coffout == 0 && (int64_t)a.n * (a.Hs / 2) * (a.Ws / 2) * a.ldout < (1ll << 31), "igemm8: pooled output layout");
      p.take_pool = true;
    }
    p.take_mask_bits = dual && !a.relu_in && a.mask && a.mask_bits && a.cout == 64 && !a.bias && a.act_out == GI_ACT_NONE && !a.stat_acc && !a.partials;
    p.take_c1w = p.take_mask_bits && a.c1w_part && a.c1w_img && mtiles % 8 == 0 && a.c1w_part_floats >= (int64_t)p.grid * 1024 &&
                 (int64_t)a.n * 16 * a.Hs * a.Ws < (1ll << 31);
    p.family = GI_FAM_IGEMM8;
    p.variant = mode == 2 ? (BN == 64 ? 7 : 6) : (dual ? 2 : mode) * 2 + (p.relu ? 1 : 0);
    p.lds_bytes = p.variant == 7 ? 2 * 22528 + 4 * 4096 : (mode == 2 ? 2 * 22528 : 2 * 20480) + 4 * 8192;
    p.lds_attr_bytes = p.lds_bytes;
    p.name = name8(p.variant);
  } else if (use6 && mode != 2 && fits31 && !(mode == 0 && a.relu_in)) {
    const int lds6 = 2 * 320 * 128 + 4 * BNk * 128;
    p.family = GI_FAM_IGEMM6;
    p.variant = (dual ? 4 : (BN == 64 ? 2 : 0) + mode) * 2 + (p.relu ? 1 : 0);
    p.lds_bytes = lds6 > epi ? lds6 : epi;
    p.lds_attr_bytes = 160 * 1024;
    p.name = name6(p.variant);
  } else {
    const int ring = 2 * (mode == 2 ? 384 : 320) * 128 + 3 * BNk * 128;
    p.family = GI_FAM_IGEMM5;
    p.variant = dual ? 6 : (BN == 64 ? 3 : 0) + mode;
    p.lds_bytes = ring > epi ? ring : epi;
    p.lds_attr_bytes = 160 * 1024;
    p.name = name5(p.variant);
  }
  return GI_OK;
}

int plan_igemm3(int mode, const IgemmArgs& a, IgemmPlan& p) {
  const int M = a.n * a.Hs * a.Ws;
  const int nph = mode == 1 ? 4 : 1;
  int BN = (a.cout % 128 == 0) ? 128 : 64;
  if (mode != 2) {
    const int tiles = ((M + 255) / 256) * (a.cout / BN) * nph;
    if (tiles < 128) return NEXT;
    if (gi_tune("GI_IGEMM3_NARROW", 1) && BN == 128 && tiles < 256) BN = 64;
  }
  GI_REQUIRE(!a.stat_acc || a.stat_pg == 0 || a.stat_pg % 256 == 0, "igemm3: stat_pg=%d must be a multiple of 256", a.stat_pg);
  const int64_t in_px = (int64_t)M * (mode == 0 ? 4 : 1), out_px = (int64_t)M * nph;
  GI_REQUIRE(in_px * a.ldin < (1ll << 31) && out_px * a.ldout < (1ll << 31), "igemm3: tensor too large for 32-bit offsets");
  p.family = GI_FAM_IGEMM3; p.mode = mode; p.bn = BN;
  p.variant = (BN == 64 ? 3 : 0) + mode;
  p.mtiles = (M + 255) / 256; p.ntiles = a.cout / BN;
  p.grid = ((p.mtiles + 7) / 8) * 8 * p.ntiles * nph;
  const int ring = 3 * (256 + BN) * 128, epi = 256 * (BN + 8) * 2 + 4 * BN * 8;
  p.lds_bytes = ring > epi ? ring : epi;
  p.lds_attr_bytes = 3 * (256 + 128) * 128;
  p.stat_to_acc = a.stat_acc != nullptr;
  p.ntiles_out = p.mtiles * nph;
  p.name = name3(p.variant);
  return GI_OK;
}

int plan_igemm7(int mode, const IgemmArgs& a, IgemmPlan& p) {
  if (a.cin % 64 != 0 || a.cout % 64 != 0) return NEXT;
  if (!gi_opt(GI_OPT_IGEMM7)) return NEXT;
  int max_split = gi_tune("GI_IGEMM7_MAXSPLIT", 8);
  if (max_split < 1) max_split = 8;
  const int M = a.n * a.Hs * a.Ws;
  const int nph = mode == 1 ? 4 : 1;
  const int mtiles = (M + 127) / 128;
  int BN = (a.cout % 128 == 0 && mtiles * (a.cout / 128) * nph >= 64) ? 128 : 64;
  {
    const int force_bn = gi_tune("GI_IGEMM7_BN", 0);
    if (force_bn == 64 || (force_bn == 128 && a.cout % 128 == 0)) BN = force_bn;
  }
  const int ntiles = a.cout / BN;
  const int tiles = mtiles * ntiles * nph;
  const int nk = (mode == 1 ? 4 : 16) * a.cin / 64;
  int splitk = (256 + tiles - 1) / tiles;
  if (splitk > max_split) splitk = max_split;
  if (splitk > nk / 8) splitk = nk / 8;
  if (splitk < 1) splitk = 1;
  const int kps = (nk + splitk - 1) / splitk;
  splitk = (nk + kps - 1) / kps;
  if (splitk > 1 && (!a.tickets || !a.ws || tiles > GI_IGEMM_TICKETS || a.ws_bytes < (int64_t)splitk * tiles * 128 * BN * 4)) return NEXT;
  constexpr int COL_TICKETS = 32;
  const int64_t out_pixels = (int64_t)M * nph;
  const int64_t col_bytes = out_pixels * BN * 2;
  p.fold = a.fold && gi_opt(GI_OPT_BN_FOLD) && a.stat_acc && a.fold->bn.groups == 1 && a.fold->bn.acc == a.stat_acc && a.tickets &&
           ntiles <= COL_TICKETS && tiles <= GI_IGEMM_TICKETS - COL_TICKETS && col_bytes <= (int64_t)gi_tune("GI_FOLD_MAX_KB", 256) * 1024 &&
           out_pixels * a.ldout * 2 < (1ll << 31) && out_pixels * a.fold->lddst * 2 < (1ll << 31) && a.ldout % 8 == 0 && a.coffout % 8 == 0 &&
           a.fold->lddst % 8 == 0 && a.fold->coffdst % 8 == 0 && (a.fold->act == GI_ACT_RELU || a.fold->act == GI_ACT_LRELU || a.fold->act == GI_ACT_NONE);
  GI_REQUIRE(!a.stat_acc || a.stat_pg == 0 || a.stat_pg % 128 == 0, "igemm7: stat_pg=%d must be a multiple of 128", a.stat_pg);
  GI_REQUIRE((int64_t)M * (mode == 0 ? 4 : 1) * a.ldin < (1ll << 31) && out_pixels * a.ldout < (1ll << 31), "igemm7: tensor too large for 32-bit offsets");
  p.family = GI_FAM_IGEMM7; p.mode = mode; p.bn = BN;
  p.variant = (BN == 64 ? 2 : 0) + mode;
  p.splitk = splitk; p.kt_per_split = kps;
  p.mtiles = mtiles; p.ntiles = ntiles;
  const int nyz = ntiles * nph * splitk;
  p.grid = mtiles >= 8 ? ((mtiles + 7) / 8) * 8 * nyz : mtiles * nyz;
  p.nstg = gi_tune("GI_IGEMM7_NSTG", 4); p.pf = gi_tune("GI_IGEMM7_PF", 1);
  if (BN == 128 || p.nstg != 6) p.nstg = 4;
  if (p.pf != 2 && p.pf != 4) p.pf = 1;
  p.nw = (p.fold || gi_opt(GI_OPT_IGEMM7_WAVES) == 4) ? 4 : 8;
  const int ring = p.nstg * (128 + BN) * 128, epi = 128 * (BN + 8) * 2 + 4 * BN * 8;
  p.lds_bytes = ring > epi ? ring : epi;
  p.lds_attr_bytes = 144 * 1024;
  p.stat_to_acc = a.stat_acc != nullptr;
  p.ntiles_out = mtiles * nph;
  p.name = name7(p.variant + (p.fold ? 4 : 0));
  return GI_OK;
}

int plan_generic(int dtype, int mode, const IgemmArgs& a, IgemmPlan& p) {
  if (dtype != GI_F16 && dtype != GI_F32) { gi_set_error("igemm: bad dtype %d", dtype); return GI_ERR_INVALID; }
  const bool f16 = dtype == GI_F16;
  const int EPC = f16 ? 8 : 4, BK = 8 * EPC;
  GI_REQUIRE(a.cin % BK == 0, "igemm: cin=%d must be a multiple of %d", a.cin, BK);
  GI_REQUIRE(a.cout % 64 == 0, "igemm: cout=%d must be a multiple of 64", a.cout);
  GI_REQUIRE(a.ldin % EPC == 0 && a.coffin % EPC == 0 && a.ldout % EPC == 0 && a.coffout % EPC == 0,
             "igemm: leading dims / channel offsets must be 16-byte aligned");
  const int phases = mode ? 4 : 1, M = a.n * a.Hs * a.Ws;
  const int nk = (mode ? 4 : 16) * a.cin / BK;
  const int64_t in_elems = (int64_t)M * (mode ? 1 : 4) * a.ldin, out_pixels = (int64_t)M * phases;
  GI_REQUIRE(in_elems < (1ll << 31) && out_pixels * a.ldout < (1ll << 31), "igemm: tensor too large for 32-bit offsets");
  const bool wide = (a.cout % 128 == 0);
  int BM = wide ? 128 : 256, BN = wide ? 128 : 64;
  int mt = (M + BM - 1) / BM, nt = a.cout / BN;
  int tiles = mt * nt * phases;
  int splitk = 1;
  int fix_max = gi_tune("GI_IGEMM_FIX_MAXSPLIT", 8);
  if (fix_max < 2) fix_max = 8;
  bool fixup = gi_opt(GI_OPT_IGEMM_FIXUP) && a.tickets && a.ws && a.force_splitk == 0 && tiles < 256 && nk >= 8;
  bool half_n = false;
  if (fixup) {
    if (wide && tiles * fix_max < 256) { half_n = true; BN = 64; nt = a.cout / BN; tiles = mt * nt * phases; }
    splitk = (256 + tiles - 1) / tiles;
    if (splitk > fix_max) splitk = fix_max;
    if (splitk > nk / 4) splitk = nk / 4;
    if (splitk < 1) splitk = 1;
    if (tiles > GI_IGEMM_TICKETS || a.ws_bytes < (int64_t)splitk * tiles * BM * BN * 4) {
      fixup = false; splitk = 1;
      if (half_n) { half_n = false; BN = 128; nt = a.cout / BN; tiles = mt * nt * phases; }
    }
  }
  if (fixup) {
  } else if (a.force_splitk > 0) splitk = a.force_splitk;
  else if (tiles < 256 && nk >= 8) {
    splitk = (gi_tune("GI_IGEMM_SPLIT_BLOCKS", 384) + tiles - 1) / tiles;
    if (splitk > nk / 4) splitk = nk / 4;
    if (splitk > 64) splitk = 64;
    if (splitk < 1) splitk = 1;
  }
  if (splitk > 1 && (a.ws == nullptr || a.ws_bytes < out_pixels * a.cout * 4)) splitk = 1;
  p.kt_per_split = (nk + splitk - 1) / splitk;
  p.splitk = (nk + p.kt_per_split - 1) / p.kt_per_split;
  p.fixup = fixup && p.splitk > 1;
  p.finish_launch = p.splitk > 1 && !p.fixup;
  p.atomics_ws = p.finish_launch && a.ws_bytes < (int64_t)p.splitk * out_pixels * a.cout * 4;
  GI_REQUIRE(!a.stat_acc || a.stat_pg == 0 || a.stat_pg % 256 == 0, "igemm: stat_pg=%d must be a multiple of 256", a.stat_pg);
  p.family = GI_FAM_GENERIC; p.mode = mode ? 1 : 0; p.bn = BN; p.BM = BM; p.half_n = half_n;
  p.mtiles = mt; p.ntiles = nt; p.grid = mt * nt * phases * p.splitk;
  p.stat_to_acc = a.stat_acc != nullptr;
  p.ntiles_out = mt * phases;
  if (p.finish_launch) {
    const int RL = 256 / (a.cout / 4) > 0 ? 256 / (a.cout / 4) : 1;
    int rpb = 64;
    while (rpb > RL && (out_pixels + rpb - 1) / rpb < 256) rpb >>= 1;
    if (rpb < RL) rpb = RL;
    GI_REQUIRE(a.cout <= 1024, "igemm split-K finish: cout=%d > 1024", a.cout);
    p.finish_rows = rpb; p.finish_blocks = (int)((out_pixels + rpb - 1) / rpb);
    p.stat_to_acc = a.stat_acc && !a.partials;
    p.ntiles_out = p.finish_blocks;
  }
  p.name = f16 ? (p.fixup ? "igemm<f16,fixup>" : (p.splitk > 1 ? "igemm<f16,splitk>" : "igemm<f16>"))
               : (p.fixup ? "igemm<f32,fixup>" : (p.splitk > 1 ? "igemm<f32,splitk>" : "igemm<f32>"));
  return GI_OK;
}

}

int gi_igemm_plan(int dtype, int mode, const IgemmArgs& a, IgemmPlan* p) {
  *p = IgemmPlan{};
  const bool dma = mode == 2 || (dtype == GI_F16 && a.force_splitk == 0 && gi_opt(GI_OPT_IGEMM_VARIANT) >= 3);
  int rc = NEXT;
  if (dma && a.cin % 64 == 0 && a.cout % 64 == 0 && a.cin <= 2048) {
    const int use5 = gi_opt(GI_OPT_IGEMM5);
    if ((mode == 1 && (use5 & 1)) || (mode == 0 && (use5 & 2)) || (mode == 2 && (use5 & 4))) rc = plan_halo(mode, a, *p);
    if (rc == NEXT) rc = plan_igemm3(mode, a, *p);
  }
  if (rc == NEXT && mode == 2) return GI_ERR_UNSUPPORTED;
  if (rc == NEXT && dma) rc = plan_igemm7(mode, a, *p);
  if (rc == NEXT) rc = plan_generic(dtype, mode, a, *p);
  return rc;
}

int op_igemm(hipStream_t st, int dtype, int mode, IgemmArgs& a) {
  IgemmPlan p;
  GI_TRY(gi_igemm_plan(dtype, mode, a, &p));
  switch (p.family) {
    case GI_FAM_IGEMM3: GI_TRY(launch_igemm3(st, p, a)); break;
    case GI_FAM_IGEMM5: case GI_FAM_IGEMM6: GI_TRY(launch_igemm5(st, p, a)); break;
    case GI_FAM_IGEMM7: GI_TRY(launch_igemm7(st, p, a)); break;
    case GI_FAM_IGEMM8: GI_TRY(launch_igemm8(st, p, a)); break;
    default: GI_TRY(launch_igemm(st, dtype, p, a)); break;
  }
  gi_note_kernel(p.name);
  if (p.fold) gi_note_fold();
  gi_igemm_returns(p, a);
  return GI_OK;
}

void gi_igemm_returns(const IgemmPlan& p, IgemmArgs& a) {
  a.stat_used = p.stat_to_acc ? 1 : 0;
  a.ntiles_out = p.ntiles_out;
  if (p.family == GI_FAM_IGEMM7) a.fold_applied = p.fold ? 1 : 0;
  if (p.family == GI_FAM_IGEMM5 || p.family == GI_FAM_IGEMM6 || p.family == GI_FAM_IGEMM8) {
    if (p.take_mask) a.mask_applied = 1;
    if (p.take_bwd) a.bwd_applied = 1;
    a.c1w_applied = p.take_c1w ? 1 : 0; a.c1w_blocks = p.take_c1w ? p.grid : 0;
    a.pool_applied = p.take_pool ? 1 : 0;
  }
}
```

### gan-inpainting_amd/csrc/net.hip

```cpp
#include <string>
#include <vector>
#include <string.h>

#include "common.h"
#include "stat_acc.h"

namespace {

struct TensorDesc {
  std::string name;
  int kind;
  int64_t shape[4];
  int ndim;
  int64_t offset, numel;
};

struct Conv {
  int ca = 0, cb = 0;
  int64_t w_off = -1, bias_off = -1;
  int64_t packed_off = -1, phase_off = -1;
  int64_t inf_off = -1;
};
struct BN {
  int c = 0;
// ... 1303 lines not shown
  const int nd = net->nd, dt = net->dtype, train = net->train;
  if (net->norm_kind != 0) return unet_forward_plain(net, s, x, y, n);
  if (!train && net->inference && nd >= 3) return unet_forward_inference(net, s, x, y, n);
  net->slot_inference[s] = 0;
  if (train) ++net->affine_gen;
  net->slot_n[s] = n;
  net->slot_train[s] = train;
  const bool fuse_u2 = nd >= 3 && net->out_c == 1 && net->fuse_head && op_c1_affine_ok(dt, 2 * net->ch[1], net->Wk[1], 2 * net->ch[1], 0);
  net->slot_fused_u2[s] = fuse_u2 ? 1 : 0;
  GI_TRY(op_c1_gather(st, dt, x, net->params + net->conv[1].w_off, concat_buf(net, s, 1), n, net->Hk[1], net->Wk[1], net->ch[1], 2 * net->ch[1], 0,
                      GI_ACT_LRELU, 1.f, nullptr, gi_opt(GI_OPT_MASK_BITS) ? (unsigned long long*)net->slot(s, net->oBits1) : nullptr, &net->slot_bits1[s]));
  bool x_saved = false;
  for (int k = 2; k < nd; ++k) {
    const int64_t pix = (int64_t)n * net->Hk[k] * net->Wk[k];
    void* R = net->slot(s, net->oR[k]);
    StatPlan sp = stat_plan(net, net->dnorm[k], pix, (pix + 127) / 128, train);
    const bool offer = sp.use && dt == GI_F16;
    IgemmFold fold;
    if (offer) fold = fold_offer(net, s, net->dnorm[k], sp, pix, skip_half(net, s, k), GI_ACT_LRELU);
    Gemm g = gemm_args(net, skip_half(net, s, k - 1), packed_ptr(net, net->conv[k]), sl(R, net->ch[k]), n, net->Hk[k], net->Wk[k]);
    with_stats(net, g, sp, offer ? &fold : nullptr);
    GI_TRY(gemm_run(net, 0, g));
    if (g.a.fold_applied) { bn_acc_commit(net, s, net->dnorm[k], sp); continue; }
    BnOpts o;
    if (k == 2) o.side = input_side_copy(net, s, x, n, sp);
    GI_TRY(bn_forward(net, s, net->dnorm[k], R, pix, g.a.ntiles_out, skip_half(net, s, k), GI_ACT_LRELU, train, sp, o));
    if (o.side.bytes > 0) x_saved = true;
  }
  {
    Gemm g = gemm_args(net, skip_half(net, s, nd - 1), packed_ptr(net, net->conv[nd]), up_input(net, s, nd), n, net->Hk[nd], net->Wk[nd]);
    g.a.act_out = GI_ACT_RELU;
    GI_TRY(gemm_run(net, 0, g));
  }
  BnAccArgs u2_acc;
  bool u2_deferred = false;
  if (!x_saved) GI_TRY(input_copy(net, s, x, n));
  for (int k = nd; k >= 2; --k) {
    const int64_t pix = (int64_t)n * net->Hk[k] * net->Wk[k], opix = 4 * pix;
    void* U = net->slot(s, net->oU[k]);
    StatPlan sp = stat_plan(net, net->unorm[k], pix, (pix + 127) / 128 * 4, train);
    Dropout drop;
    GI_TRY(dropout_prepare(net, s, k, n, true, drop));
    const bool fused = (k == 2) && fuse_u2;
    const bool offer = sp.use && dt == GI_F16 && !fused;
    IgemmFold fold;
    if (offer) fold = fold_offer(net, s, net->unorm[k], sp, opix, up_half(net, s, k - 1), GI_ACT_RELU, drop);
    Gemm g = gemm_args(net, up_input(net, s, k), phase_ptr(net, net->up[k]), sl(U, net->ch[k - 1]), n, net->Hk[k], net->Wk[k]);
    if (k < nd) { g.a.relu_in = 1; g.a.relu_cend = net->ch[k]; }
    with_stats(net, g, sp, offer ? &fold : nullptr);
    GI_TRY(gemm_run(net, 1, g));
    if (g.a.fold_applied) { bn_acc_commit(net, s, net->unorm[k], sp); continue; }
    if (drop.p > 0.f && !sp.use) GI_TRY(dropout_draw(net, drop, opix * net->ch[k - 1]));
    if (fused && sp.use) {
      u2_acc = bn_acc_args(net, s, net->unorm[k], sp, opix, 1);
      bn_acc_commit(net, s, net->unorm[k], sp);
      u2_deferred = true;
      continue;
    }
    BnOpts o;
    o.apply = !fused; o.drop = drop;
    GI_TRY(bn_forward(net, s, net->unorm[k], U, opix, g.a.ntiles_out, up_half(net, s, k - 1), GI_ACT_RELU, train, sp, o));
  }
  C1Affine aff = u2_affine(net, s);
  if (u2_deferred) aff.bn = &u2_acc;
  return head_forward(net, s, y, n, true, fuse_u2 ? &aff : nullptr);
}

int unet_backward(gi_net* net, int s, const float* dy, float* dx, int need_wgrad, int phase) {
  if (net->norm_kind != 0) return unet_backward_plain(net, s, dy, dx, need_wgrad, phase);
  const int nd = net->nd, n = net->slot_n[s];
  GI_REQUIRE(n > 0 && (net->slot_train[s] || !need_wgrad), "unet_backward: slot %d holds no train-mode forward", s);
  GI_REQUIRE(!net->slot_inference[s], "unet_backward: slot %d holds an inference forward (gi_net_set_inference): nothing was saved for a backward", s);
  GI_REQUIRE(net->out_c == 1 || !need_wgrad, "unet_backward: parameter gradients of a %d-channel generator are not built", net->out_c);
  const int evalbn = net->slot_train[s] ? 0 : 1;
  net->bwd_eval = evalbn;
  auto gC = [&](int k) { return (void*)net->shared(net->ogC[k]); };
  auto gA = [&](int k) { return (void*)net->shared(net->ogA[k]); };
  auto dropped = [&](int k) { return !evalbn && net->dropout_p > 0.f && k >= 5 && k <= nd - 1; };
  void* D = nullptr;
  if (phase == 0 || phase == 1) {
    C1Affine aff = u2_affine(net, s);
    GI_TRY(head_backward(net, s, dy, need_wgrad, net->slot_fused_u2[s] ? &aff : nullptr));
    GI_TRY(clear_pending_bwd(net, &net->unorm[2], nd - 1));
    for (int k = 1; k <= nd - 1; ++k) {
      const int kk = k + 1, ck = net->ch[k], ca = net->up[kk].ca;
      const int64_t pix = (int64_t)n * net->Hk[k] * net->Wk[k];
      D = side_dz(net);
      BwdFuse& pend = net->bwd_pending[net->unorm[kk].id];
      ActBnBwdArgs b = act_bwd_args(up_half(net, s, k), pix, GI_ACT_NONE);
      set_g2(b, sl(gC(k), ck, 2 * ck, ck));
      b.x = net->slot(s, net->oU[kk]);
      if (dropped(kk)) b.drop_scale = 1.f / (1.f - net->dropout_p);
      GI_TRY(act_bn_bwd(net, s, b, D, &net->unorm[kk], need_wgrad, &pend));
      pend = BwdFuse();
      if (need_wgrad) {
        WgradArgs wa = wgrad_args(net, up_input(net, s, kk), sl(D, ck), n, net->Hk[kk], net->Wk[kk], net->grads + net->up[kk].w_off);
        wa.relu_S = kk < nd ? 1 : 0;
        GI_TRY(wgrad_run(net, wa));
      }
      void* gout = (kk == nd) ? (void*)net->shared(net->ogE) : gC(kk);
      Gemm g = gemm_args(net, sl(D, ck), packed_ptr(net, net->up[kk]), sl(gout, ca), n, net->Hk[kk], net->Wk[kk]);
      const int kn = kk + 1;
      if (kk <= nd - 1 && !dropped(kn)) {
        const int64_t pixn = (int64_t)n * net->Hk[kk] * net->Wk[kk];
        BwdFuse& bf = net->bwd_pending[net->unorm[kn].id];
        bf = bwd_fuse_plan(net, s, net->unorm[kn], net->slot(s, net->oU[kn]), pixn, pixn / 256, 0.f);
        bf.c0 = ca / 2; bf.c = ca / 2;
        with_bn_bwd(g, bf);
      }
      GI_TRY(gemm_run(net, 0, g));
    }
  }
  if (phase == 1) return GI_OK;
  const bool run_inner = phase != 4, run_outer = phase != 3;
  int lrelu1_done = 0;
  C1WFuse c1w;
  if (run_inner) {
    const int c = net->ch[nd], cb = net->ch[nd - 1];
    D = side_dz(net);
    ActBnBwdArgs b = act_bwd_args(up_input(net, s, nd), (int64_t)n * net->Hk[nd] * net->Wk[nd], GI_ACT_NONE);
    set_g2(b, sl(net->shared(net->ogE), c));
    GI_TRY(act_bn_bwd(net, s, b, D));
    if (need_wgrad)
      GI_TRY(wgrad_run(net, wgrad_args(net, sl(D, c), skip_half(net, s, nd - 1), n, net->Hk[nd], net->Wk[nd], net->grads + net->conv[nd].w_off)));
    GI_TRY(gemm_run(net, 1, gemm_args(net, sl(D, c), phase_ptr(net, net->conv[nd]), sl(gA(nd - 1), cb), n, net->Hk[nd], net->Wk[nd])));
  }
  for (int k = nd - 1; k >= 2; --k) {
    if (k >= 5 ? !run_inner : !run_outer) continue;
    const int c = net->ch[k], cb = net->ch[k - 1];
    D = side_dz(net);
    ActBnBwdArgs b = act_bwd_args(skip_half(net, s, k), (int64_t)n * net->Hk[k] * net->Wk[k], GI_ACT_LRELU);
    set_g1(b, sl(gA(k), c));
    set_g2(b, sl(gC(k), c, 2 * c));
    b.x = net->slot(s, net->oR[k]);
    GI_TRY(act_bn_bwd(net, s, b, D, &net->dnorm[k], need_wgrad));
    if (need_wgrad)
      GI_TRY(wgrad_run(net, wgrad_args(net, sl(D, c), skip_half(net, s, k - 1), n, net->Hk[k], net->Wk[k], net->grads + net->conv[k].w_off)));
    Gemm g = gemm_args(net, sl(D, c), phase_ptr(net, net->conv[k]), sl(gA(k - 1), cb), n, net->Hk[k], net->Wk[k]);
    if (k == 2) {
      with_first_layer_bwd(net, s, g, skip_half(net, s, 1), need_wgrad, dx != nullptr, c1w);
      g.a.add = gC(1); g.a.ldadd = 2 * cb;
    }
    GI_TRY(gemm_run(net, 1, g));
    if (k == 2) lrelu1_done = g.a.mask_applied;
  }
  if (run_outer) {
    const int c = net->ch[1];
    ActBnBwdArgs a1 = act_bwd_args(skip_half(net, s, 1), (int64_t)n * net->Hk[1] * net->Wk[1], GI_ACT_LRELU);
    set_g1(a1, sl(gA(1), c));
    set_g2(a1, sl(gC(1), c, 2 * c));
    GI_TRY(first_layer_tail(net, s, net->conv[1], n, net->Hk[1], net->Wk[1], a1, need_wgrad, dx, lrelu1_done, &c1w));
  }
  return GI_OK;
}

int unet_forward_plain(gi_net* net, int s, const float* x, float* y, int n) {
  hipStream_t st = net->ctx->stream;
  const int nd = net->nd, dt = net->dtype, train = net->train;
  net->slot_inference[s] = 0;
  net->slot_n[s] = n;
  net->slot_train[s] = train;
  net->slot_fused_u2[s] = 0;
  GI_TRY(input_copy(net, s, x, n));
  GI_TRY(op_c1_gather(st, dt, x, net->params + net->conv[1].w_off, concat_buf(net, s, 1), n, net->Hk[1], net->Wk[1], net->ch[1], 2 * net->ch[1], 0,
                      GI_ACT_LRELU, 1.f, conv_bias(net, net->conv[1])));
  for (int k = 2; k < nd; ++k) {
    void* R = net->slot(s, net->oR[k]);
    Gemm g = gemm_args(net, skip_half(net, s, k - 1), packed_ptr(net, net->conv[k]), sl(R, net->ch[k]), n, net->Hk[k], net->Wk[k]);
    g.a.bias = conv_bias(net, net->conv[k]);
    GI_TRY(gemm_run(net, 0, g));
    GI_TRY(plain_norm_forward(net, s, net->dnorm[k], R, n, net->Hk[k] * net->Wk[k], skip_half(net, s, k), GI_ACT_LRELU));
  }
  {
    Gemm g = gemm_args(net, skip_half(net, s, nd - 1), packed_ptr(net, net->conv[nd]), up_input(net, s, nd), n, net->Hk[nd], net->Wk[nd]);
    g.a.act_out = GI_ACT_RELU; g.a.bias = conv_bias(net, net->conv[nd]);
    GI_TRY(gemm_run(net, 0, g));
  }
  for (int k = nd; k >= 2; --k) {
    void* U = net->slot(s, net->oU[k]);
    Dropout drop;
    GI_TRY(dropout_prepare(net, s, k, n, false, drop));
    Gemm g = gemm_args(net, up_input(net, s, k), phase_ptr(net, net->up[k]), sl(U, net->ch[k - 1]), n, net->Hk[k], net->Wk[k]);
    if (k < nd) { g.a.relu_in = 1; g.a.relu_cend = net->ch[k]; }
    g.a.bias = conv_bias(net, net->up[k]);
    GI_TRY(gemm_run(net, 1, g));
    GI_TRY(plain_norm_forward(net, s, net->unorm[k], U, n, net->Hk[k - 1] * net->Wk[k - 1], up_half(net, s, k - 1), GI_ACT_RELU, drop));
  }
  return head_forward(net, s, y, n, true);
}

int plain_norm_backward(gi_net* net, int s, const BN& b, ActBnBwdArgs a, void* dx, int n, int hw) {
  if (net->norm_kind != 1) {
    a.x = nullptr;
    return act_bn_bwd(net, s, a, dx);
  }
  a.dx = dx;
  return op_act_in_bwd(net->ctx->stream, net->dtype, a, n, hw, (const float*)net->slot(s, net->oInStats) + b.in_off);
}

int unet_backward_plain(gi_net* net, int s, const float* dy, float* dx, int need_wgrad, int phase) {
  const int nd = net->nd, n = net->slot_n[s];
  GI_REQUIRE(n > 0, "unet_backward: slot %d holds no forward", s);
  GI_REQUIRE(net->out_c == 1 || !need_wgrad, "unet_backward: parameter gradients of a %d-channel generator are not built", net->out_c);
  net->bwd_eval = 0;
  auto gC = [&](int k) { return (void*)net->shared(net->ogC[k]); };
  auto gA = [&](int k) { return (void*)net->shared(net->ogA[k]); };
  void* D = net->shared(net->oD);
  const bool dropped = net->slot_train[s] && net->dropout_p > 0.f;
  if (phase == 0 || phase == 1) {
    GI_TRY(head_backward(net, s, dy, need_wgrad));
    for (int k = 1; k <= nd - 1; ++k) {
      const int kk = k + 1, ck = net->ch[k], ca = net->up[kk].ca;
      const int64_t pix = (int64_t)n * net->Hk[k] * net->Wk[k];
      ActBnBwdArgs b = act_bwd_args(up_half(net, s, k), pix, GI_ACT_NONE);
      set_g2(b, sl(gC(k), ck, 2 * ck, ck));
      b.x = net->slot(s, net->oU[kk]);
      if (dropped && kk >= 5 && kk <= nd - 1) b.drop_scale = 1.f / (1.f - net->dropout_p);
      GI_TRY(plain_norm_backward(net, s, net->unorm[kk], b, D, n, net->Hk[k] * net->Wk[k]));
      if (need_wgrad) {
        GI_TRY(bias_grad(net, net->up[kk], D, pix, ck));
        WgradArgs wa = wgrad_args(net, up_input(net, s, kk), sl(D, ck), n, net->Hk[kk], net->Wk[kk], net->grads + net->up[kk].w_off);
        wa.relu_S = kk < nd ? 1 : 0;
        GI_TRY(wgrad_run(net, wa));
      }
// ... 459 lines not shown
```

### include/ganinpaint.h

```cpp
#ifndef GANINPAINT_H
#define GANINPAINT_H

#include <stddef.h>
#include <stdint.h>

#ifdef __cplusplus
extern "C" {
#endif

typedef enum {
  GI_OK = 0,
  GI_ERR_INVALID = -1,
  GI_ERR_HIP = -2,
  GI_ERR_STATE = -3,
  GI_ERR_UNSUPPORTED = -4
} gi_status;

typedef enum { GI_F32 = 0, GI_F16 = 1 } gi_dtype;
typedef enum { GI_ACT_NONE = 0, GI_ACT_RELU = 1, GI_ACT_LRELU = 2 } gi_act;

typedef struct gi_ctx gi_ctx;
typedef struct gi_net gi_net;

const char* gi_last_error(void);
int gi_version(void);

int gi_set_option(const char* name, int value);
int gi_get_option(const char* name, int* value);
const char* gi_debug_last_kernel(void);
int gi_debug_fold_count(void);

int gi_ctx_create(int device_id, void* hip_stream, gi_ctx** out);
int gi_ctx_destroy(gi_ctx* ctx);
int gi_ctx_sync(gi_ctx* ctx);

int gi_unet_create(gi_ctx* ctx, int num_downs, int ngf, float dropout_p, int H, int W, int max_n,
                   int dtype, int n_slots, gi_net** out);
int gi_unet_create_ex(gi_ctx* ctx, int num_downs, int ngf, int out_c, float dropout_p, int H, int W,
                      int max_n, int dtype, int n_slots, gi_net** out);
int gi_unet_create_norm(gi_ctx* ctx, int num_downs, int ngf, int out_c, int norm_kind, float dropout_p, int H,
                        int W, int max_n, int dtype, int n_slots, gi_net** out);
int gi_unet_create_padded(gi_ctx* ctx, int num_downs, int ngf, int ch1, int out_c, int norm_kind, float dropout_p,
                          int H, int W, int max_n, int dtype, int n_slots, gi_net** out);
int gi_patchgan_create(gi_ctx* ctx, int H, int W, int sigmoid, int max_n, int dtype, int n_slots,
                       gi_net** out);
int gi_patchgan_create_sn(gi_ctx* ctx, int H, int W, int sigmoid, int spectral_norm, int n_power_iterations, int max_n,
                          int dtype, int n_slots, gi_net** out);
int gi_net_sn_read(gi_net* net, int slot, float* sigma6, float* eff_params, int64_t count);
int gi_dcgan_create(gi_ctx* ctx, int H, int W, int max_n, int dtype, int n_slots, gi_net** out);
int gi_dcgan_debug_forward_convs(gi_net* net, int slot, const float* x, int n);
int gi_net_destroy(gi_net* net);

int gi_net_tensor_count(gi_net* net);
int gi_net_tensor_desc(gi_net* net, int index, char* name, int name_cap, int* kind, int64_t* shape4,
                       int* ndim, int64_t* offset, int64_t* numel);
int64_t gi_net_param_floats(gi_net* net);
int64_t gi_net_buffer_floats(gi_net* net);
int64_t gi_net_workspace_bytes(gi_net* net);
int gi_net_bind(gi_net* net, float* params, float* grads, float* buffers, void* workspace,
                int64_t workspace_bytes);
int gi_net_sync_weights(gi_net* net);
int gi_net_set_train(gi_net* net, int train);
int gi_net_set_inference(gi_net* net, int inference);
int gi_net_set_loss_scale(gi_net* net, float scale);
int gi_net_set_bn_groups(gi_net* net, int groups);
int gi_net_set_dropout_seed(gi_net* net, uint64_t seed);
int gi_net_get_dropout_state(gi_net* net, uint64_t* seed, uint64_t* counter);
int gi_net_set_dropout_state(gi_net* net, uint64_t seed, uint64_t counter);
int gi_net_dropout_mask(gi_net* net, int slot, int level, uint8_t* out_nchw, int64_t count);
int gi_net_set_dropout_mask(gi_net* net, int slot, int level, const uint8_t* mask_nchw);

int gi_net_saved_activation(gi_net* net, int slot, int kind, int level, float* out_nchw, int64_t count);
int gi_net_debug_nonzero_tickets(gi_net* net, int* count);

int gi_net_forward(gi_net* net, int slot, const float* x, float* y, int n);
int gi_net_backward(gi_net* net, int slot, const float* dy, float* dx, int need_wgrad);

int gi_net_backward_phase(gi_net* net, int slot, const float* dy, float* dx, int need_wgrad, int phase);
int64_t gi_net_phase_split(gi_net* net);
int64_t gi_net_phase_split2(gi_net* net);

typedef struct gi_comm gi_comm;
int gi_comm_unique_id(char* id128_host);
int gi_comm_create(const char* id128_host, int rank, int world, int device_id, gi_comm** out);
int gi_comm_destroy(gi_comm* comm);
int gi_allreduce_sum_f32(gi_comm* comm, float* buf, int64_t count, void* hip_comm_stream);
int gi_net_allreduce_grads_async(gi_net* net, gi_comm* comm, int64_t begin, int64_t end, void* hip_comm_stream);
int gi_allreduce_wait(gi_comm* comm, void* hip_comm_stream, void* hip_compute_stream);

int gi_patchgan_gradient_penalty(gi_net* net, const float* xhat, int n, float lam, float* penalty_out);
int gi_patchgan_gp_saved_activation(gi_net* net, int level, float* out_nchw, int64_t count);
int gi_interpolate(gi_ctx* ctx, const float* real, const float* fake, const float* eps, int n, int64_t hw, float* out);

int gi_mask_apply(gi_ctx* ctx, const float* ground, const float* mask, float* mask_c, float* masked,
                  int64_t count, int flags);
int gi_mask_composite(gi_ctx* ctx, const float* masked, const float* gen, const float* mask_c,
                      float* inpainted, int64_t count);
int gi_mul(gi_ctx* ctx, const float* a, const float* b, float* out, int64_t count);
int gi_add(gi_ctx* ctx, const float* a, const float* b, float* out, int64_t count, float alpha);

int gi_loss_l1(gi_ctx* ctx, const float* a, const float* b, int64_t count, float* loss_out,
               float* grad_a, float gscale, float* scratch);
int gi_loss_rmse(gi_ctx* ctx, const float* a, const float* b, int64_t count, float eps, float* loss_out,
                 float* grad_a, float gscale, float* scratch);
int gi_loss_mse(gi_ctx* ctx, const float* a, const float* b, int64_t count, float* loss_out,
                float* grad_a, float gscale, float* scratch);
int gi_loss_local(gi_ctx* ctx, const float* yhat, const float* y, const float* mask, int64_t count,
                  int kind, float* loss_out, float* grad_yhat, float gscale, float* scratch);
int gi_loss_adv(gi_ctx* ctx, const float* pred, int n, int kind, float target, float* loss_out,
                float* grad_pred, float gscale);
int gi_loss_adv_pair(gi_ctx* ctx, const float* pred2, int n_each, int kind, float target_a, float target_b, float* loss_a,
                     float* loss_b, float* grad_pred2, float gscale_a, float gscale_b);

// ... 242 lines not shown
```

Baseline: 16880 images/sec.

## Fuse BN-backward reduction with skip-gradient add into U-Net encoder dgrad epilogues

Extends the fused BatchNorm-backward statistic reduction in the transposed-conv (phase mode) GEMM epilogues of igemm3, igemm5 and igemm8 so it also handles a second gradient source (the skip-connection add). The encoder backward loop now plans this fusion for layers k>2, letting the next act_bn_bwd skip a separate reduction pass over the activation. This removes a full read of the gradient and activation tensors per layer. In exchange the epilogues get extra loads, another template variant, and a debug counter.

```diff
diff --git a/gan-inpainting_amd/backend.py b/gan-inpainting_amd/backend.py
--- a/gan-inpainting_amd/backend.py
+++ b/gan-inpainting_amd/backend.py
@@ -19,6 +19,7 @@
     "gi_get_option": (_i, [C.c_char_p, C.POINTER(_i)]),
     "gi_debug_last_kernel": (C.c_char_p, []),
     "gi_debug_fold_count": (_i, []),
+    "gi_debug_bwd_reduce_count": (_i, []),
     "gi_ctx_create": (_i, [_i, _vp, C.POINTER(_vp)]),
     "gi_ctx_destroy": (_i, [_vp]),
     "gi_ctx_sync": (_i, [_vp]),
diff --git a/gan-inpainting_amd/csrc/api.hip b/gan-inpainting_amd/csrc/api.hip
--- a/gan-inpainting_amd/csrc/api.hip
+++ b/gan-inpainting_amd/csrc/api.hip
@@ -26,9 +26,10 @@
   {"GI_WGRAD_STREAM", 1, 0, 0}, {"GI_MASK_BITS", 1, 0, 0}, {"GI_C1W_FUSE", 1, 0, 0}, {"GI_IGEMM7_WAVES", 8, 0, 0},
 };
 thread_local const char* g_last_kernel = "";
-int g_fold_count = 0;
+int g_fold_count = 0, g_bwd_reduce_count = 0;
 }
 void gi_note_fold() { __atomic_fetch_add(&g_fold_count, 1, __ATOMIC_RELAXED); }
+void gi_note_bwd_reduce() { __atomic_fetch_add(&g_bwd_reduce_count, 1, __ATOMIC_RELAXED); }
 
 int gi_opt(int id) {
   OptDesc& o = g_opts[id];
@@ -63,6 +64,7 @@
 }
 const char* gi_debug_last_kernel(void) { return g_last_kernel; }
 int gi_debug_fold_count(void) { return __atomic_load_n(&g_fold_count, __ATOMIC_RELAXED); }
+int gi_debug_bwd_reduce_count(void) { return __atomic_load_n(&g_bwd_reduce_count, __ATOMIC_RELAXED); }
 
 const char* gi_last_error(void) { return g_err; }
 int gi_version(void) { return 100; }
diff --git a/gan-inpainting_amd/csrc/common.h b/gan-inpainting_amd/csrc/common.h
--- a/gan-inpainting_amd/csrc/common.h
+++ b/gan-inpainting_amd/csrc/common.h
@@ -26,6 +26,7 @@
 int gi_opt(int id);
 void gi_note_kernel(const char* name);
 void gi_note_fold();
+void gi_note_bwd_reduce();
 #ifdef GI_ABLATION
 #include <stdlib.h>
 static inline int gi_tune(const char* env, int dflt) { const char* e = getenv(env); return e ? atoi(e) : dflt; }
diff --git a/gan-inpainting_amd/csrc/elementwise.hip b/gan-inpainting_amd/csrc/elementwise.hip
--- a/gan-inpainting_amd/csrc/elementwise.hip
+++ b/gan-inpainting_amd/csrc/elementwise.hip
@@ -1478,6 +1478,7 @@
 #undef GI_RED_T
 #undef GI_RED
   GI_LAUNCH_CHECK();
+  gi_note_bwd_reduce();
   return GI_OK;
 }
 
diff --git a/gan-inpainting_amd/csrc/halo_args.h b/gan-inpainting_amd/csrc/halo_args.h
--- a/gan-inpainting_amd/csrc/halo_args.h
+++ b/gan-inpainting_amd/csrc/halo_args.h
@@ -47,7 +47,7 @@
   kp.relu_cend = a.relu_cend > 0 ? a.relu_cend : a.cin;
   kp.ntiles = p.ntiles;
   kp.mask = (const char*)a.mask; kp.ldmask = a.ldmask; kp.coffmask = a.coffmask; kp.mask_slope = a.mask_slope;
-  kp.add = a.mask ? (const char*)a.add : nullptr; kp.ldadd = a.ldadd; kp.coffadd = a.coffadd;
+  kp.add = (a.mask || p.bwd_add) ? (const char*)a.add : nullptr; kp.ldadd = a.ldadd; kp.coffadd = a.coffadd;
   if (p.take_mask_bits) kp.mask_bits = a.mask_bits;
   if (p.take_c1w) { kp.c1w_img = a.c1w_img; kp.c1w_part = a.c1w_part; kp.c1w_scale = a.c1w_scale; kp.c1w_skip_out = a.c1w_skip_out; }
   kp.bwd_c = a.cout;
diff --git a/gan-inpainting_amd/csrc/igemm3.hip b/gan-inpainting_amd/csrc/igemm3.hip
--- a/gan-inpainting_amd/csrc/igemm3.hip
+++ b/gan-inpainting_amd/csrc/igemm3.hip
@@ -23,6 +23,10 @@
   int Hin, Win, Hout, Wout;
   int mtiles, ntiles;
   int dbg;
+  const char* bwd_x; int bwd_ldx;
+  const float* bwd_scale; const float* bwd_shift; const float* bwd_mean; const float* bwd_inv;
+  float bwd_slope; unsigned long long* bwd_acc; int bwd_reps;
+  const char* add; int ldadd, coffadd;
 };
 
 
@@ -322,6 +326,68 @@
   }
   constexpr int CPRO = BN / 8;
   const int oc = tid % CPRO;
+  if constexpr (PHASE == 1 && DBG == 0) {
+    if (p.bwd_acc) {
+      constexpr int RP = NTHREADS / CPRO, NB = 4;
+      const int och = n0 + oc * 8;
+      float bsc[8], bsh[8], bmu[8], biv[8], bs[8], bsx[8];
+#pragma unroll
+      for (int e = 0; e < 8; ++e) {
+        bsc[e] = p.bwd_scale[och + e]; bsh[e] = p.bwd_shift[och + e]; bmu[e] = p.bwd_mean[och + e]; biv[e] = p.bwd_inv[och + e];
+        bs[e] = bsx[e] = 0.f;
+      }
+#pragma unroll 1
+      for (int h = 0; h < BM / (RP * NB); ++h) {
+        int opxs[NB];
+        u4_t xs[NB], ad[NB];
+#pragma unroll
+        for (int k = 0; k < NB; ++k) {
+          opxs[k] = out_pixel(m0 + tid / CPRO + (h * NB + k) * RP);
+          xs[k] = *(const u4_t*)(p.bwd_x + ((int64_t)opxs[k] * p.bwd_ldx + och) * 2);
+          ad[k] = *(const u4_t*)(p.add + ((int64_t)opxs[k] * p.ldadd + p.coffadd + och) * 2);
+        }
+#pragma unroll
+        for (int k = 0; k < NB; ++k) {
+          const int r = tid / CPRO + (h * NB + k) * RP;
+          const u4_t v = *(const u4_t*)((const char*)stg + ((int64_t)r * SLD + oc * 8) * 2);
+          const h8_t xv = __builtin_bit_cast(h8_t, xs[k]);
+          const h8_t gv = __builtin_bit_cast(h8_t, v);
+          const h8_t av = __builtin_bit_cast(h8_t, ad[k]);
+#pragma unroll
+          for (int e = 0; e < 8; ++e) {
+            const float xf = (float)xv[e];
+            const bool pos = fmaf(xf, bsc[e], bsh[e]) > 0.f;
+            const float g = (float)gv[e] + (pos ? (float)av[e] : 0.f);
+            const float dz = g * (pos ? 1.f : p.bwd_slope);
+            bs[e] += dz;
+            bsx[e] = fmaf(dz, (xf - bmu[e]) * biv[e], bsx[e]);
+          }
+          *(u4_t*)(p.out + ((int64_t)opxs[k] * p.ldout + p.coffout + och) * 2) = v;
+        }
+      }
+#pragma unroll
+      for (int e = 0; e < 8; ++e) {
+#pragma unroll
+        for (int off = CPRO; off < 64; off <<= 1) { bs[e] += __shfl_xor(bs[e], off); bsx[e] += __shfl_xor(bsx[e], off); }
+      }
+      __syncthreads();
+      float* fold = (float*)smem;
+      if (lane < CPRO) {
+#pragma unroll
+        for (int e = 0; e < 8; ++e) { fold[(wave * BN + oc * 8 + e) * 2] = bs[e]; fold[(wave * BN + oc * 8 + e) * 2 + 1] = bsx[e]; }
+      }
+      __syncthreads();
+      if (tid < BN) {
+        float s = 0.f, q = 0.f;
+#pragma unroll
+        for (int w = 0; w < NW; ++w) { s += fold[(w * BN + tid) * 2]; q += fold[(w * BN + tid) * 2 + 1]; }
+        const int rep = (mt_idx + ph) & (p.bwd_reps - 1);
+        gi_stat_add(p.bwd_acc, p.cout, rep, 0, 0, n0 + tid, s);
+        gi_stat_add(p.bwd_acc, p.cout, rep, 0, 1, n0 + tid, q);
+      }
+      return;
+    }
+  }
 #pragma unroll 1
   for (int r = tid / CPRO; r < BM; r += NTHREADS / CPRO) {
     const int m = m0 + r;
@@ -364,6 +430,14 @@
   else { kp.Hin = 2 * a.Hs; kp.Win = 2 * a.Ws; kp.Hout = a.Hs; kp.Wout = a.Ws; }
   kp.mtiles = p.mtiles;
   kp.ntiles = p.ntiles;
+  kp.bwd_x = nullptr; kp.bwd_ldx = 0; kp.bwd_scale = kp.bwd_shift = kp.bwd_mean = kp.bwd_inv = nullptr;
+  kp.bwd_slope = 1.f; kp.bwd_acc = nullptr; kp.bwd_reps = 1; kp.add = nullptr; kp.ldadd = kp.coffadd = 0;
+  if (p.take_bwd) {
+    kp.bwd_x = (const char*)a.bwd_x; kp.bwd_ldx = a.bwd_ldx;
+    kp.bwd_scale = a.bwd_scale; kp.bwd_shift = a.bwd_shift; kp.bwd_mean = a.bwd_mean; kp.bwd_inv = a.bwd_inv;
+    kp.bwd_slope = a.bwd_slope; kp.bwd_acc = a.bwd_acc; kp.bwd_reps = a.bwd_reps > 0 ? a.bwd_reps : 1;
+    kp.add = (const char*)a.add; kp.ldadd = a.ldadd; kp.coffadd = a.coffadd;
+  }
 #define GI_K3(V, MODE_, BN_, NAME) case V: return gi_launch_lds<igemm3_kernel<MODE_, BN_, 8>>(dim3(p.grid), 512, p.lds_bytes, p.lds_attr_bytes, st, kp);
 #ifdef GI_ABLATION
   { const char* e = getenv("GI_IGEMM3_DBG"); kp.dbg = e ? atoi(e) : 0; }
diff --git a/gan-inpainting_amd/csrc/igemm5.hip b/gan-inpainting_amd/csrc/igemm5.hip
--- a/gan-inpainting_amd/csrc/igemm5.hip
+++ b/gan-inpainting_amd/csrc/igemm5.hip
@@ -31,7 +31,7 @@
   }
 }
 
-template <int MODE, int BN>
+template <int MODE, int BN, bool ADD2 = false>
 __device__ __forceinline__ void epilogue5(const KP5& p, f4_t (&acc)[4][BN / 32], char* smem, int tid, int lane, int wm, int wn,
                                           int mt_idx, int nt_idx, int ph, int py, int px, int n0, int img, int y0, int x0, int lgTW) {
   constexpr bool DUAL = MODE == 3;
@@ -114,56 +114,94 @@
     }
   }
   constexpr int NR = BM / (512 / CPRO);
-  int opxs[NR];
-  u4_t mk[NR], ad[NR], xs[NR];
   const int och = n0 + (DUAL ? (oc & 7) : oc) * 8;
-#pragma unroll
-  for (int k = 0; k < NR; ++k) {
-    const int r = tid / CPRO + k * (512 / CPRO);
-    opxs[k] = out_pixel(r) + (DUAL ? (oc >> 3) : 0);
-    const int64_t opx = opxs[k];
-    if (p.mask) mk[k] = *(const u4_t*)(p.mask + (opx * p.ldmask + p.coffmask + och) * 2);
-    if (p.mask && p.add) ad[k] = *(const u4_t*)(p.add + (opx * p.ldadd + p.coffadd + och) * 2);
-    if (bwd) xs[k] = *(const u4_t*)(p.bwd_x + (opx * p.bwd_ldx + och) * 2);
-  }
-#pragma unroll
-  for (int k = 0; k < NR; ++k) {
-    const int r = tid / CPRO + k * (512 / CPRO);
-    const int64_t opx = opxs[k];
-    const int64_t o = opx * p.ldout + p.coffout + och;
-    u4_t v = *(const u4_t*)((const char*)stg + ((int64_t)r * SLD + oc * 8) * 2);
-    if (bwd) {
-      const h8_t xv = __builtin_bit_cast(h8_t, xs[k]);
-      const h8_t gv = __builtin_bit_cast(h8_t, v);
-#pragma unroll
-      for (int e = 0; e < 8; ++e) {
-        const float xf = (float)xv[e];
-        const float dz = (float)gv[e] * (fmaf(xf, bsc[e], bsh[e]) > 0.f ? 1.f : p.bwd_slope);
-        bs[e] += dz;
-        bsx[e] = fmaf(dz, (xf - bmu[e]) * biv[e], bsx[e]);
-      }
-    }
-    if (p.mask) {
-      const h8_t m = __builtin_bit_cast(h8_t, mk[k]);
-      h8_t hv = __builtin_bit_cast(h8_t, v);
-      if (p.add) {
-        const h8_t a8 = __builtin_bit_cast(h8_t, ad[k]);
+  bool copied = false;
+  if constexpr (ADD2) {
+    if (bwd && !p.mask && p.add) {
+      constexpr int NB = 4, RP = 512 / CPRO;
+#pragma unroll 1
+      for (int h = 0; h < BM / (RP * NB); ++h) {
+        int opx4[NB];
+        u4_t x4[NB], a4[NB];
+#pragma unroll
+        for (int k = 0; k < NB; ++k) {
+          opx4[k] = out_pixel(tid / CPRO + (h * NB + k) * RP);
+          x4[k] = *(const u4_t*)(p.bwd_x + ((int64_t)opx4[k] * p.bwd_ldx + och) * 2);
+          a4[k] = *(const u4_t*)(p.add + ((int64_t)opx4[k] * p.ldadd + p.coffadd + och) * 2);
+        }
+#pragma unroll
+        for (int k = 0; k < NB; ++k) {
+          const int r = tid / CPRO + (h * NB + k) * RP;
+          const u4_t v = *(const u4_t*)((const char*)stg + ((int64_t)r * SLD + oc * 8) * 2);
+          const h8_t xv = __builtin_bit_cast(h8_t, x4[k]);
+          const h8_t gv = __builtin_bit_cast(h8_t, v);
+          const h8_t av = __builtin_bit_cast(h8_t, a4[k]);
+#pragma unroll
+          for (int e = 0; e < 8; ++e) {
+            const float xf = (float)xv[e];
+            const bool pos = fmaf(xf, bsc[e], bsh[e]) > 0.f;
+            const float g = (float)gv[e] + (pos ? (float)av[e] : 0.f);
+            const float dz = g * (pos ? 1.f : p.bwd_slope);
+            bs[e] += dz;
+            bsx[e] = fmaf(dz, (xf - bmu[e]) * biv[e], bsx[e]);
+          }
+          *(u4_t*)(p.out + ((int64_t)opx4[k] * p.ldout + p.coffout + och) * 2) = v;
+        }
+      }
+      copied = true;
+    }
+  }
+  if (!copied) {
+    int opxs[NR];
+    u4_t mk[NR], ad[NR], xs[NR];
+#pragma unroll
+    for (int k = 0; k < NR; ++k) {
+      const int r = tid / CPRO + k * (512 / CPRO);
+      opxs[k] = out_pixel(r) + (DUAL ? (oc >> 3) : 0);
+      const int64_t opx = opxs[k];
+      if (p.mask) mk[k] = *(const u4_t*)(p.mask + (opx * p.ldmask + p.coffmask + och) * 2);
+      if (p.mask && p.add) ad[k] = *(const u4_t*)(p.add + (opx * p.ldadd + p.coffadd + och) * 2);
+      if (bwd) xs[k] = *(const u4_t*)(p.bwd_x + (opx * p.bwd_ldx + och) * 2);
+    }
+#pragma unroll
+    for (int k = 0; k < NR; ++k) {
+      const int r = tid / CPRO + k * (512 / CPRO);
+      const int64_t opx = opxs[k];
+      const int64_t o = opx * p.ldout + p.coffout + och;
+      u4_t v = *(const u4_t*)((const char*)stg + ((int64_t)r * SLD + oc * 8) * 2);
+      if (bwd) {
+        const h8_t xv = __builtin_bit_cast(h8_t, xs[k]);
+        const h8_t gv = __builtin_bit_cast(h8_t, v);
 #pragma unroll
         for (int e = 0; e < 8; ++e) {
-          const bool pos = (float)m[e] > 0.f;
-          const float g = (float)hv[e] + (pos ? (float)a8[e] : 0.f);
-          hv[e] = (half_t)(pos ? g : g * p.mask_slope);
-        }
-      } else {
-#pragma unroll
-        for (int e = 0; e < 8; ++e) hv[e] = (float)m[e] > 0.f ? hv[e] : (half_t)((float)hv[e] * p.mask_slope);
-      }
-      v = __builtin_bit_cast(u4_t, hv);
-    }
+          const float xf = (float)xv[e];
+          const float dz = (float)gv[e] * (fmaf(xf, bsc[e], bsh[e]) > 0.f ? 1.f : p.bwd_slope);
+          bs[e] += dz;
+          bsx[e] = fmaf(dz, (xf - bmu[e]) * biv[e], bsx[e]);
+        }
+      }
+      if (p.mask) {
+        const h8_t m = __builtin_bit_cast(h8_t, mk[k]);
+        h8_t hv = __builtin_bit_cast(h8_t, v);
+        if (p.add) {
+          const h8_t a8 = __builtin_bit_cast(h8_t, ad[k]);
+#pragma unroll
+          for (int e = 0; e < 8; ++e) {
+            const bool pos = (float)m[e] > 0.f;
+            const float g = (float)hv[e] + (pos ? (float)a8[e] : 0.f);
+            hv[e] = (half_t)(pos ? g : g * p.mask_slope);
+          }
+        } else {
+#pragma unroll
+          for (int e = 0; e < 8; ++e) hv[e] = (float)m[e] > 0.f ? hv[e] : (half_t)((float)hv[e] * p.mask_slope);
+        }
+        v = __builtin_bit_cast(u4_t, hv);
+      }
 #ifdef GI_ABLATION
-    if (p.dbg_epi & 1) { *(u4_t*)(p.out + ((o * 2) & 0xFFF0)) = v; continue; }
+      if (p.dbg_epi & 1) { *(u4_t*)(p.out + ((o * 2) & 0xFFF0)) = v; continue; }
 #endif
-    *(u4_t*)(p.out + o * 2) = v;
+      *(u4_t*)(p.out + o * 2) = v;
+    }
   }
   if (bwd) {
     static_assert(DUAL || CPRO == 16 || CPRO == 8, "CPRO");
@@ -636,7 +674,7 @@
     if (t == 12345.678f) p.out[0] = 1;
     return;
   }
-  epilogue5<MODE, BN>(p, acc, smem, tid, lane, wm, wn, mt_idx, nt_idx, ph, py, px, n0, img, y0, x0, lgTW);
+  epilogue5<MODE, BN, (MODE == 1 && BN == 128 && !RELU)>(p, acc, smem, tid, lane, wm, wn, mt_idx, nt_idx, ph, py, px, n0, img, y0, x0, lgTW);
 }
 
 }
diff --git a/gan-inpainting_amd/csrc/igemm8.hip b/gan-inpainting_amd/csrc/igemm8.hip
--- a/gan-inpainting_amd/csrc/igemm8.hip
+++ b/gan-inpainting_amd/csrc/igemm8.hip
@@ -10,7 +10,7 @@
   __builtin_amdgcn_raw_ptr_buffer_load_lds(rs, (__attribute__((address_space(3))) void*)lds_wave_base, 16, voff, soff, 0, 0);
 }
 
-template <int MODE, int BN, bool BITS>
+template <int MODE, int BN, bool BITS, bool ADD2>
 __device__ __forceinline__ void epilogue8(const KP5& p, f4_t (&acc)[4][BN / 16], char* smem, int tid, int lane, int wave, int mt_idx,
                                           int ph, int py, int px, int n0, int img, int y0, int x0, int lgTW) {
   constexpr bool DUAL = MODE == 3;
@@ -205,8 +205,43 @@
       copied = true;
     }
   }
+  if constexpr (ADD2) {
+    if (bwd && !p.mask && p.add) {
+      constexpr int NB = 4;
+#pragma unroll 1
+      for (int h = 0; h < BM / (RP * NB); ++h) {
+        int opxs[NB];
+        u4_t xs[NB], ad[NB];
+#pragma unroll
+        for (int k = 0; k < NB; ++k) {
+          opxs[k] = out_pixel(tid / CPRO + (h * NB + k) * RP);
+          xs[k] = *(const u4_t*)(p.bwd_x + ((int64_t)opxs[k] * p.bwd_ldx + och - p.bwd_c0) * 2);
+          ad[k] = *(const u4_t*)(p.add + ((int64_t)opxs[k] * p.ldadd + p.coffadd + och) * 2);
+        }
+#pragma unroll
+        for (int k = 0; k < NB; ++k) {
+          const int r = tid / CPRO + (h * NB + k) * RP;
+          const u4_t v = *(const u4_t*)((const char*)stg + ((int64_t)r * SLD + oc * 8) * 2);
+          const h8_t xv = __builtin_bit_cast(h8_t, xs[k]);
+          const h8_t gv = __builtin_bit_cast(h8_t, v);
+          const h8_t av = __builtin_bit_cast(h8_t, ad[k]);
+#pragma unroll
+          for (int e = 0; e < 8; ++e) {
+            const float xf = (float)xv[e];
+            const bool pos = fmaf(xf, bsc[e], bsh[e]) > 0.f;
+            const float g = (float)gv[e] + (pos ? (float)av[e] : 0.f);
+            const float dz = g * (pos ? 1.f : p.bwd_slope);
+            bs[e] += dz;
+            bsx[e] = fmaf(dz, (xf - bmu[e]) * biv[e], bsx[e]);
+          }
+          *(u4_t*)(p.out + ((int64_t)opxs[k] * p.ldout + p.coffout + och) * 2) = v;
+        }
+      }
+      copied = true;
+    }
+  }
   if constexpr (!DUAL && MODE != 2) {
-    if (bwd && !p.mask) {
+    if (bwd && !p.mask && !copied) {
       constexpr int NB = 4;
 #pragma unroll 1
       for (int h = 0; h < BM / (RP * NB); ++h) {
@@ -357,8 +392,9 @@
   }
 }
 
-template <int MODE, bool RELU, int DBG = 0, int BN = 128>
+template <int MODE, bool RELU, int DBG = 0, int BN = 128, bool ADD2 = false>
 __global__ void __launch_bounds__(256, 2) igemm8_kernel(KP5 p) {
+  static_assert(!ADD2 || (MODE == 1 && !RELU && BN == 128), "two gradient sources: the sub-pixel-phase kernel without the input ReLU");
   static_assert(BN == 128 || (BN == 64 && MODE != 3), "64-column tiles: not with both px phases in one tile");
   static_assert(MODE >= 0 && MODE <= 3, "modes 0 (stride-2 gather), 1 (phase), 2 (3x3 / s1), 3 (both px phases)");
   static_assert(!(MODE == 2 && RELU), "the 3x3 mode has no fused input ReLU");
@@ -652,7 +688,7 @@
     if (t == 12345.678f) p.out[0] = 1;
     return;
   }
-  epilogue8<MODE, BN, (MODE == 3 && !RELU)>(p, acc, smem, tid, lane, wave, mt_idx, ph, py, px, n0, img, y0, x0, lgTW);
+  epilogue8<MODE, BN, (MODE == 3 && !RELU), ADD2>(p, acc, smem, tid, lane, wave, mt_idx, ph, py, px, n0, img, y0, x0, lgTW);
 }
 
 }
@@ -677,6 +713,7 @@
   }
 #undef GI_K8D
 #endif
+  if (p.bwd_add && p.variant == 2) return gi_launch_lds<igemm8_kernel<1, false, 0, 128, true>>(grid, 256, p.lds_bytes, p.lds_attr_bytes, st, kp);
   switch (p.variant) { GI_IGEMM8_KERNELS(GI_K8) }
 #undef GI_K8
   return GI_ERR_INVALID;
diff --git a/gan-inpainting_amd/csrc/igemm_plan.h b/gan-inpainting_amd/csrc/igemm_plan.h
--- a/gan-inpainting_amd/csrc/igemm_plan.h
+++ b/gan-inpainting_amd/csrc/igemm_plan.h
@@ -13,6 +13,7 @@
   int splitk, kt_per_split;
   bool fixup, finish_launch, atomics_ws;
   bool fold, take_mask, take_mask_bits, take_c1w, take_bwd, bwd_range, take_pool, stat_to_acc;
+  bool bwd_add;
   int TH, TW, mtiles, ntiles, grid, lds_bytes, lds_attr_bytes, ntiles_out;
   int finish_rows, finish_blocks;
   const char* name;
diff --git a/gan-inpainting_amd/csrc/igemm_plan.hip b/gan-inpainting_amd/csrc/igemm_plan.hip
--- a/gan-inpainting_amd/csrc/igemm_plan.hip
+++ b/gan-inpainting_amd/csrc/igemm_plan.hip
@@ -46,11 +46,16 @@
   const bool take8 = use8 && (mode != 2 || (TW == 32 && !a.relu_in)) && (dual || BN == 128 || mode == 2) && a.cin % (mode == 0 ? 64 : 32) == 0 && TW >= 16 &&
       fits31 && !(mode == 0 && a.relu_in) && (use8 >= 2 || p.grid >= gi_tune("GI_IGEMM8_MINGRID", 512));
   p.bwd_range = a.bwd_c > 0 && (a.bwd_c0 != 0 || a.bwd_c != a.cout);
-  if (a.bwd_acc && !a.mask && mode != 2 && a.cout % 128 == 0 && BN == 128 && (!p.bwd_range || (take8 && a.bwd_c0 % 128 == 0 && a.bwd_c % 128 == 0 && a.bwd_c0 + a.bwd_c <= a.cout))) {
+  const bool add2 = a.bwd_acc && a.add && !a.mask;
+  const bool add2_ok = mode == 1 && !a.relu_in && !p.bwd_range && (take8 || (use6 && fits31)) && a.ldadd % 8 == 0 && a.coffadd % 8 == 0 &&
+                       out_px * a.ldadd < (1ll << 31);
+  if (a.bwd_acc && !a.mask && mode != 2 && a.cout % 128 == 0 && BN == 128 && (!add2 || add2_ok) &&
+      (!p.bwd_range || (take8 && a.bwd_c0 % 128 == 0 && a.bwd_c % 128 == 0 && a.bwd_c0 + a.bwd_c <= a.cout))) {
     const int64_t px_per_tile = 256 * (mode == 1 ? 4 : 1);
     GI_REQUIRE(a.bwd_ldx % 8 == 0 && out_px * a.bwd_ldx < (1ll << 31) && (a.bwd_pg == 0 || a.bwd_pg % px_per_tile == 0) && a.coffout == 0,
                "igemm5: fused BatchNorm-backward reduction: layout");
     p.take_bwd = true;
+    p.bwd_add = add2;
   }
   if (take8) {
     if (mode == 2 && a.pool2 && !a.mask && !a.stat_acc && !a.partials) {
@@ -105,6 +110,11 @@
   p.stat_to_acc = a.stat_acc != nullptr;
   p.ntiles_out = p.mtiles * nph;
   p.name = name3(p.variant);
+  if (mode == 1 && a.bwd_acc && a.add && !a.mask && !a.relu_in && M % 256 == 0 && a.bwd_pg == 0 && (a.bwd_c == 0 || (a.bwd_c0 == 0 && a.bwd_c == a.cout)) &&
+      a.bwd_ldx % 8 == 0 && out_px * a.bwd_ldx < (1ll << 31) && a.ldadd % 8 == 0 && a.coffadd % 8 == 0 && out_px * a.ldadd < (1ll << 31)) {
+    p.take_bwd = true;
+    p.bwd_add = true;
+  }
   return GI_OK;
 }
 
@@ -262,6 +272,7 @@
   a.stat_used = p.stat_to_acc ? 1 : 0;
   a.ntiles_out = p.ntiles_out;
   if (p.family == GI_FAM_IGEMM7) a.fold_applied = p.fold ? 1 : 0;
+  if (p.family == GI_FAM_IGEMM3 && p.take_bwd) a.bwd_applied = 1;
   if (p.family == GI_FAM_IGEMM5 || p.family == GI_FAM_IGEMM6 || p.family == GI_FAM_IGEMM8) {
     if (p.take_mask) a.mask_applied = 1;
     if (p.take_bwd) a.bwd_applied = 1;
diff --git a/gan-inpainting_amd/csrc/net.hip b/gan-inpainting_amd/csrc/net.hip
--- a/gan-inpainting_amd/csrc/net.hip
+++ b/gan-inpainting_amd/csrc/net.hip
@@ -1409,6 +1409,7 @@
     C1Affine aff = u2_affine(net, s);
     GI_TRY(head_backward(net, s, dy, need_wgrad, net->slot_fused_u2[s] ? &aff : nullptr));
     GI_TRY(clear_pending_bwd(net, &net->unorm[2], nd - 1));
+    GI_TRY(clear_pending_bwd(net, &net->dnorm[2], nd - 2));
     for (int k = 1; k <= nd - 1; ++k) {
       const int kk = k + 1, ck = net->ch[k], ca = net->up[kk].ca;
       const int64_t pix = (int64_t)n * net->Hk[k] * net->Wk[k];
@@ -1460,13 +1461,21 @@
     set_g1(b, sl(gA(k), c));
     set_g2(b, sl(gC(k), c, 2 * c));
     b.x = net->slot(s, net->oR[k]);
-    GI_TRY(act_bn_bwd(net, s, b, D, &net->dnorm[k], need_wgrad));
+    BwdFuse& pend = net->bwd_pending[net->dnorm[k].id];
+    GI_TRY(act_bn_bwd(net, s, b, D, &net->dnorm[k], need_wgrad, &pend));
+    pend = BwdFuse();
     if (need_wgrad)
       GI_TRY(wgrad_run(net, wgrad_args(net, sl(D, c), skip_half(net, s, k - 1), n, net->Hk[k], net->Wk[k], net->grads + net->conv[k].w_off)));
     Gemm g = gemm_args(net, sl(D, c), phase_ptr(net, net->conv[k]), sl(gA(k - 1), cb), n, net->Hk[k], net->Wk[k]);
     if (k == 2) {
       with_first_layer_bwd(net, s, g, skip_half(net, s, 1), need_wgrad, dx != nullptr, c1w);
       g.a.add = gC(1); g.a.ldadd = 2 * cb;
+    } else {
+      const int64_t pix = (int64_t)n * net->Hk[k] * net->Wk[k];
+      BwdFuse& bf = net->bwd_pending[net->dnorm[k - 1].id];
+      bf = bwd_fuse_plan(net, s, net->dnorm[k - 1], net->slot(s, net->oR[k - 1]), pix * 4, pix / 256 * 4, 0.2f);
+      with_bn_bwd(g, bf);
+      if (bf.planned) { g.a.add = gC(k - 1); g.a.ldadd = 2 * cb; }
     }
     GI_TRY(gemm_run(net, 1, g));
     if (k == 2) lrelu1_done = g.a.mask_applied;
diff --git a/include/ganinpaint.h b/include/ganinpaint.h
--- a/include/ganinpaint.h
+++ b/include/ganinpaint.h
@@ -29,6 +29,7 @@
 int gi_get_option(const char* name, int* value);
 const char* gi_debug_last_kernel(void);
 int gi_debug_fold_count(void);
+int gi_debug_bwd_reduce_count(void);
 
 int gi_ctx_create(int device_id, void* hip_stream, gi_ctx** out);
 int gi_ctx_destroy(gi_ctx* ctx);
```

New measurement: 16970 images/sec (median of 6 runs). Within noise of the previous version (+0.5%).
